# mp3guy/ElasticFusion

Hardware: AMD Instinct MI355X
Metric: frames/s per GPU, 640x480 3-level ICP+fuse (higher is better)
Workload: dtype f32

## Files before the change

### elasticfusion_amd/api.py

```python
from __future__ import annotations

import ctypes as C
import os
import re

import numpy as np

_HERE = os.path.dirname(os.path.abspath(__file__))
LIB_PATH = os.environ.get("EF_HIP_LIB") or os.path.join(_HERE, "libefusion_hip.so")
_lib = None

c_f, c_i, c_u32, P = C.c_float, C.c_int, C.c_uint32, C.c_void_p


class EFError(RuntimeError):
    pass


class ef_config(C.Structure):
    _fields_ = [("width", c_i), ("height", c_i), ("fx", c_f), ("fy", c_f), ("cx", c_f), ("cy", c_f),
                ("time_delta", c_i), ("confidence", c_f), ("depth_cut", c_f), ("icp_weight", c_f),
                ("fast_odom", c_i), ("so3", c_i), ("frame_to_frame_rgb", c_i), ("pyramid", c_i), ("rgb_only", c_i),
                ("close_loops", c_i), ("max_surfels", c_u32), ("device", c_i), ("stream", P)]

# ... 1147 lines not shown

    def _carveArgs(self, depths, poses, params, among, kw):
        T = self.get_T_wc().reshape(1, 16) if poses is None else np.ascontiguousarray(poses, np.float64).reshape(-1, 16)
        if params is None:
            if not isinstance(depths, DevBuf) and "width" not in kw and "height" not in kw:
                kw = dict(kw, width=int(np.shape(depths)[-1]), height=int(np.shape(depths)[-2]))
            params = self.carveParams(**kw)
        else:
            assert not kw, "give params or keywords, not both"
        if isinstance(depths, DevBuf):
            assert len(T) * params.width * params.height * 2 <= depths.nbytes, (len(T), depths.nbytes)
            keep, dp = depths, depths.p
        else:
            keep = np.ascontiguousarray(depths, np.uint16).reshape(-1, params.height, params.width)
            assert len(keep) == len(T), (keep.shape, T.shape)
            dp = _ptr(keep)
        views = ef_carve_views(len(T), _ptr(T), dp)
        if isinstance(among, dict):
            among = self.mapSelection(**among)
        return params, views, (C.byref(among) if among is not None else None), (T, keep, among)

    def carveSelect(self, depths, poses=None, params: ef_carve_params | None = None, among=None, max_rows: int | None = None,
                    count: bool = False, votes: bool = False, **kw):
        params, views, pa, keep = self._carveArgs(depths, poses, params, among, kw)
        n = self.lastCount() if max_rows is None or votes else 0
        cap = n if max_rows is None else int(max_rows)
        rows = np.zeros(max(cap, 1), np.uint32)
        v2 = np.zeros((max(n, 1), 2), np.uint8) if votes else None
        total = c_u32(0)
        _chk(lib().ef_map_carve_select(self.h, C.byref(params), C.byref(views), pa, _ptr(rows) if cap else None, cap, C.byref(total),
                                       _ptr(v2) if votes else None), self.h)
        out = (rows[:min(cap, total.value)].copy(),) + ((total.value,) if count else ()) + ((v2[:n],) if votes else ())
        return out if len(out) > 1 else out[0]

    def carveSelectDevice(self, depths_dev, poses, params: ef_carve_params, among, rows_dev, max_rows: int, count_dev, votes_dev=None):
        T = np.ascontiguousarray(poses, np.float64).reshape(-1, 16)
        if isinstance(among, dict):
            among = self.mapSelection(**among)
        views = ef_carve_views(len(T), _ptr(T), _dev(depths_dev))
        _chk(lib().ef_map_carve_select_dev(self.h, C.byref(params), C.byref(views), C.byref(among) if among is not None else None,
                                           _dev(rows_dev), int(max_rows), _dev(count_dev), _dev(votes_dev)), self.h)

    def carveSurfels(self, depths, poses=None, params: ef_carve_params | None = None, among=None, **kw) -> dict:
        params, views, pa, keep = self._carveArgs(depths, poses, params, among, kw)
        res = ef_carve_result()
        fn = lib().ef_map_carve_dev if isinstance(depths, DevBuf) else lib().ef_map_carve
        _chk(fn(self.h, C.byref(params), C.byref(views), pa, C.byref(res)), self.h)
        return {k: int(getattr(res, k)) for k, _ in ef_carve_result._fields_}

    def setReferenceDownload(self, on=True):
        _chk(lib().ef_set_reference_download(self.h, int(on)), self.h)

    def uploadMap(self, surfels: np.ndarray):
        s = np.ascontiguousarray(surfels, np.float32).reshape(-1, 12)
        _chk(lib().ef_map_upload(self.h, _ptr(s), len(s)), self.h)

    def getPoseQT(self) -> np.ndarray:
        qt = np.zeros(7, np.float64)
        _chk(lib().ef_get_pose_qt(self.h, _ptr(qt)), self.h)
        return qt

    def checkpoint(self, last_rgb, last_depth) -> dict:
        return dict(map=self.downloadMap(), tick=self.getTick(), qt=self.getPoseQT(), rgb=np.ascontiguousarray(last_rgb, np.uint8).copy(),
                    depth=np.ascontiguousarray(last_depth, np.uint16).copy())

    def restore(self, ck: dict):
        self.uploadMap(ck["map"])
        qt = np.ascontiguousarray(ck["qt"], np.float64).reshape(7)
        _chk(lib().ef_restore_state(self.h, int(ck["tick"]), _ptr(qt), _ptr(ck["rgb"]), _ptr(ck["depth"])), self.h)

    def savePly(self, path: str):
        _chk(lib().ef_save_ply(self.h, path.encode()), self.h)

    def saveFreiburg(self, path: str):
        _chk(lib().ef_save_freiburg(self.h, path.encode()), self.h)

    def setRgbOnly(self, v): _chk(lib().ef_set_rgb_only(self.h, int(v)), self.h)
    def setIcpWeight(self, v): _chk(lib().ef_set_icp_weight(self.h, v), self.h)
    def setPyramid(self, v): _chk(lib().ef_set_pyramid(self.h, int(v)), self.h)
    def setFastOdom(self, v): _chk(lib().ef_set_fast_odom(self.h, int(v)), self.h)
    def setSo3(self, v): _chk(lib().ef_set_so3(self.h, int(v)), self.h)
    def setFrameToFrameRGB(self, v): _chk(lib().ef_set_frame_to_frame_rgb(self.h, int(v)), self.h)
    def setConfidenceThreshold(self, v): _chk(lib().ef_set_confidence_threshold(self.h, v), self.h)
    def setDepthCutoff(self, v): _chk(lib().ef_set_depth_cutoff(self.h, v), self.h)
    def setInputOverlap(self, on): _chk(lib().ef_set_input_overlap(self.h, int(on)), self.h)
    def setInputCuMask(self, one_in_n): _chk(lib().ef_set_input_cu_mask(self.h, int(one_in_n)), self.h)
    def setDeformation(self, graph, isFern=False):
        g = np.ascontiguousarray(graph, np.float32).reshape(-1, 16)
        _chk(lib().ef_set_deformation(self.h, _ptr(g), len(g), int(isFern)), self.h)

    def setGraphReplay(self, on): _chk(lib().ef_set_graph_replay(self.h, int(on)), self.h)

    def image(self, name: str) -> np.ndarray:
        which, dt, ch = self.IMAGES[name]
        W, H = self.cfg.width, self.cfg.height
        out = np.zeros((H, W, ch) if ch > 1 else (H, W), dt)
        _chk(lib().ef_get_image(self.h, which, _ptr(out), out.nbytes), self.h)
        return out

    def trackerBuffer(self, name: str, level: int = 0, tracker: int = 0) -> np.ndarray:
        which, dt, planes = self.TRACKER[name]
        w, h = self.cfg.width >> level, self.cfg.height >> level
        out = np.zeros((h * planes, w), dt)
        _chk(lib().ef_get_tracker_buffer_of(self.h, tracker, which, level, _ptr(out), out.nbytes), self.h)
        return out

    def enableTiming(self, on=True):
        _chk(lib().ef_enable_timing(self.h, int(on)), self.h)

    def timings(self) -> dict:
        arr = (ef_timing * 32)()
        n = c_i(0)
        _chk(lib().ef_get_timings(self.h, arr, 32, C.byref(n)), self.h)
        return {arr[i].name.decode(): arr[i].ms for i in range(n.value)}


class ops:
    @staticmethod
    def _f32(a):
        return np.ascontiguousarray(a, np.float32)

    @staticmethod
    def _image_op(name, src, dtype, scale, *scalars):
        h, w = src.shape[:2]
        shape = (h // scale, w // scale)
        s, d = DevBuf.from_array(src), DevBuf(shape[0] * shape[1] * np.dtype(dtype).itemsize)
        _chk(getattr(lib(), "ef_op_" + name)(s.p, w, h, *scalars, d.p, None))
        return d.to_array(dtype, shape)

    @staticmethod
    def pyr_down(src):
        return ops._image_op("pyr_down", src, np.uint16, 2)

    @staticmethod
    def create_vmap(depth, fx, fy, cx, cy, cutoff, init=None):
        h, w = depth.shape
        d = DevBuf.from_array(depth)
        v = DevBuf.from_array(np.zeros((3 * h, w), np.float32) if init is None else init)
        k = ef_intr(fx, fy, cx, cy)
        _chk(lib().ef_op_create_vmap(C.byref(k), d.p, w, h, cutoff, v.p, None))
        return v.to_array(np.float32, (3 * h, w))

    @staticmethod
    def create_nmap(vmap, init=None):
        h3, w = vmap.shape
        v = DevBuf.from_array(vmap)
        n = DevBuf.from_array(np.zeros((h3, w), np.float32) if init is None else init)
        _chk(lib().ef_op_create_nmap(v.p, w, h3 // 3, n.p, None))
        return n.to_array(np.float32, (h3, w))

    @staticmethod
    def transform_maps(vmap, nmap, R, t):
        h3, w = vmap.shape
        v, n = DevBuf.from_array(vmap), DevBuf.from_array(nmap)
        R9, t3 = ops._f32(R).reshape(9), ops._f32(t).reshape(3)
        _chk(lib().ef_op_transform_maps(v.p, n.p, w, h3 // 3, _ptr(R9), _ptr(t3), v.p, n.p, None))
        return v.to_array(np.float32, (h3, w)), n.to_array(np.float32, (h3, w))

    @staticmethod
    def copy_maps(vtex, ntex):
        h, w, _ = vtex.shape
        v4, n4 = DevBuf.from_array(ops._f32(vtex)), DevBuf.from_array(ops._f32(ntex))
        tmp, vm, nm = DevBuf(h * w * 16), DevBuf(h * w * 12), DevBuf(h * w * 12)
        _chk(lib().ef_op_copy_maps(v4.p, n4.p, w, h, tmp.p, vm.p, nm.p, None))
        return tmp.to_array(np.float32, (h, w, 4)), vm.to_array(np.float32, (3 * h, w)), nm.to_array(np.float32, (3 * h, w))

    @staticmethod
    def resize_map(src, normalize, init=None):
        h3, w = src.shape
        s = DevBuf.from_array(src)
        o = DevBuf.from_array(np.zeros((h3 // 2, w // 2), np.float32) if init is None else init)
        fn = lib().ef_op_resize_nmap if normalize else lib().ef_op_resize_vmap
        _chk(fn(s.p, w, h3 // 3, o.p, None))
        return o.to_array(np.float32, (h3 // 2, w // 2))

    @staticmethod
    def pyr_down_gauss_f(src):
        return ops._image_op("pyr_down_gauss_f", src, np.float32, 2)

    @staticmethod
    def pyr_down_uchar_gauss(src):
        return ops._image_op("pyr_down_uchar_gauss", src, np.uint8, 2)

    @staticmethod
    def vertices_to_depth(vmaps_tmp, cutoff):
        return ops._image_op("vertices_to_depth", ops._f32(vmaps_tmp), np.float32, 1, cutoff)

    @staticmethod
    def bgr_to_intensity(rgba):
        return ops._image_op("image_bgr_to_intensity", rgba, np.uint8, 1)

    @staticmethod
    def derivative_images(img):
        h, w = img.shape
        s, dx, dy = DevBuf.from_array(img), DevBuf(h * w * 2), DevBuf(h * w * 2)
        _chk(lib().ef_op_compute_derivative_images(s.p, w, h, dx.p, dy.p, None))
        return dx.to_array(np.int16, (h, w)), dy.to_array(np.int16, (h, w))

    @staticmethod
    def project_to_point_cloud(depth, fx, fy, cx, cy, level=0):
        h, w = depth.shape
        s, d = DevBuf.from_array(depth), DevBuf(h * w * 12)
        k = ef_intr(fx, fy, cx, cy)
        _chk(lib().ef_op_project_to_point_cloud(s.p, w, h, C.byref(k), level, d.p, None))
        return d.to_array(np.float32, (h, w, 3))

    @staticmethod
    def icp_step(Rcurr, tcurr, vmap_curr, nmap_curr, Rprev_inv, tprev, intr, vmap_g_prev, nmap_g_prev, distThres, angleThres):
        h3, w = vmap_curr.shape
        bufs = [DevBuf.from_array(a) for a in (vmap_curr, nmap_curr, vmap_g_prev, nmap_g_prev)]
        A, b, res = np.zeros((6, 6), np.float32), np.zeros(6, np.float32), np.zeros(2, np.float32)
        k = ef_intr(*intr)
        _chk(lib().ef_op_icp_step(_ptr(ops._f32(Rcurr).reshape(9)), _ptr(ops._f32(tcurr)), bufs[0].p, bufs[1].p,
                                  _ptr(ops._f32(Rprev_inv).reshape(9)), _ptr(ops._f32(tprev)), C.byref(k), bufs[2].p, bufs[3].p,
                                  distThres, angleThres, w, h3 // 3, _ptr(A), _ptr(b), _ptr(res), None))
        return A, b, res

    @staticmethod
    def rgb_residual(minScale, dIdx, dIdy, lastDepth, nextDepth, lastImage, nextImage, maxDepthDelta, kt, krkinv):
        h, w = nextImage.shape
        bufs = [DevBuf.from_array(a) for a in (dIdx, dIdy, lastDepth, nextDepth, lastImage, nextImage)]
        corres = DevBuf(h * w * 16)
        sigma, count = c_i(0), c_i(0)
        _chk(lib().ef_op_compute_rgb_residual(minScale, bufs[0].p, bufs[1].p, bufs[2].p, bufs[3].p, bufs[4].p, bufs[5].p, corres.p,
                                              maxDepthDelta, _ptr(ops._f32(kt)), _ptr(ops._f32(krkinv).reshape(9)), w, h,
                                              C.byref(sigma), C.byref(count), None))
        return corres.to_array(DATATERM, (h, w)), sigma.value, count.value

    @staticmethod
    def rgb_step(corres, sigma, cloud, fx, fy, dIdx, dIdy, sobelScale):
        h, w = corres.shape
        bufs = [DevBuf.from_array(a) for a in (corres, ops._f32(cloud), dIdx, dIdy)]
        A, b = np.zeros((6, 6), np.float32), np.zeros(6, np.float32)
        _chk(lib().ef_op_rgb_step(bufs[0].p, sigma, bufs[1].p, fx, fy, bufs[2].p, bufs[3].p, sobelScale, w, h,
                                  _ptr(A), _ptr(b), None))
        return A, b

    @staticmethod
    def so3_step(lastImage, nextImage, imageBasis, kinv, krlr):
        h, w = nextImage.shape
        li, ni = DevBuf.from_array(lastImage), DevBuf.from_array(nextImage)
        A, b, res = np.zeros((3, 3), np.float32), np.zeros(3, np.float32), np.zeros(2, np.float32)
        _chk(lib().ef_op_so3_step(li.p, ni.p, _ptr(ops._f32(imageBasis).reshape(9)), _ptr(ops._f32(kinv).reshape(9)),
                                  _ptr(ops._f32(krlr).reshape(9)), w, h, _ptr(A), _ptr(b), _ptr(res), None))
        return A, b, res

    @staticmethod
    def model_maps(pred_vertex, pred_normal, fill_vertex, fill_normal, R, t, maxDepthRGB=6.0, pred_image=None, fill_image=None, camera_frame=False,
                   force_fill_image=False, tally=False, dense_count=0, dense_samples=1, joint=False, raw=None, rgb=None, depth_cut=3.0, init=None):
        h, w, _ = pred_vertex.shape
        init = init or {}
        keep = [DevBuf.from_array(ops._f32(a)) for a in (pred_vertex, pred_normal, fill_vertex, fill_normal)]
        a = ef_model_maps_op()
        a.cols, a.rows = w, h
        a.pred_vertex, a.pred_normal, a.fill_vertex, a.fill_normal = (b.p for b in keep)
        if pred_image is not None:
            imgs = [DevBuf.from_array(np.ascontiguousarray(i, np.uint8)) for i in (pred_image, fill_image)]
            keep += imgs
            a.pred_image, a.fill_image = imgs[0].p, imgs[1].p
        a.R[:] = [float(v) for v in ops._f32(R).reshape(9)]
        a.t[:] = [float(v) for v in ops._f32(t).reshape(3)]
        a.max_depth_rgb = float(maxDepthRGB)
        a.camera_frame, a.force_fill_image, a.tally = int(camera_frame), int(force_fill_image), int(tally)
        a.dense_count, a.dense_samples = int(dense_count), int(dense_samples)
        spec = {}
        for l in range(3):
            spec[f"vmap{l}"] = spec[f"nmap{l}"] = (np.float32, (3 * (h >> l), w >> l))
        spec["depth0"], spec["last0"] = (np.float32, (h, w)), (np.uint8, (h, w))
        if joint:
            spec.update(filtered=(np.uint16, (h, w)), metric=(np.float32, (h, w)), metric_filtered=(np.float32, (h, w)), next0=(np.uint8, (h, w)))
        out = {}
        for name, (dt, shp) in spec.items():
            start = np.zeros(shp, dt) if name not in init else np.ascontiguousarray(init[name], dt)
            assert start.shape == shp, (name, start.shape, shp)
            out[name] = DevBuf.from_array(start)
        for l in range(3):
            a.vmap[l], a.nmap[l] = out[f"vmap{l}"].p, out[f"nmap{l}"].p
        a.depth0, a.last0 = out["depth0"].p, out["last0"].p
        if joint:
            fr = [DevBuf.from_array(np.ascontiguousarray(raw, np.uint16)), DevBuf.from_array(np.ascontiguousarray(rgb, np.uint8))]
            assert raw.shape == (h, w) and rgb.shape == (h, w, 3)
            keep += fr
            a.joint, a.raw, a.rgb3, a.depth_cut = 1, fr[0].p, fr[1].p, float(depth_cut)
            a.filtered, a.metric, a.metric_filtered, a.next0 = (out[n].p for n in ("filtered", "metric", "metric_filtered", "next0"))
        left = C.c_uint(0)
        _chk(lib().ef_op_model_maps(C.byref(a), C.byref(left), None))
        res = {name: out[name].to_array(*spec[name]) for name in spec}
        res["dense_count"] = int(left.value)
        return res

    @staticmethod
    def sobel_mask(nextImage, nextDepth):
        h, w = nextImage[0].shape
        img = [DevBuf.from_array(np.ascontiguousarray(a, np.uint8)) for a in nextImage]
        dep = [DevBuf.from_array(ops._f32(a)) for a in nextDepth]
        for l in range(3):
            assert nextImage[l].shape == nextDepth[l].shape == (h >> l, w >> l), (l, nextImage[l].shape, nextDepth[l].shape)
        outs = [[DevBuf((h >> l) * (w >> l) * sz, fill=0xA5) for l in range(3)] for sz in (2, 2, 1, 4)]
        arr = lambda bufs: (P * 3)(*[b.p for b in bufs])
        _chk(lib().ef_op_sobel_mask(arr(img), arr(dep), w, h, arr(outs[0]), arr(outs[1]), arr(outs[2]), arr(outs[3]), None))
        return tuple([b.to_array(dt, (h >> l, w >> l)) for l, b in enumerate(bufs)] for bufs, dt in zip(outs, (np.int16, np.int16, np.uint8, np.uint32)))

    @staticmethod
    def clean_deform(cam, T_wc, time, idx, vc, ct, nr, confThreshold, timeDelta, maxDepth, surfels, newUnstable, graph, depth, isFern=0):
        s = ops._f32(surfels).reshape(-1, 12)
        nu = ops._f32(newUnstable).reshape(-1, 12)
        g = ops._f32(graph).reshape(-1, 16)
        bufs = [DevBuf.from_array(a) for a in (idx, ops._f32(vc), ops._f32(ct), ops._f32(nr), g, ops._f32(depth))]
        sb, nb = DevBuf.from_array(s), DevBuf.from_array(nu if len(nu) else np.zeros((1, 12), np.float32))
        out = DevBuf((len(s) + len(nu) + 1) * 48)
        n = c_u32(0)
        _chk(lib().ef_op_clean_deform(C.byref(cam), _ptr(ops._T(T_wc)), time, bufs[0].p, bufs[1].p, bufs[2].p, bufs[3].p,
                                      confThreshold, timeDelta, maxDepth, sb.p, len(s), nb.p, len(nu),
                                      bufs[4].p, len(g), bufs[5].p, int(isFern), out.p, C.byref(n), None))
        return out.to_array(np.float32, (n.value, 12))

    LINALG = dict(ldlt6=0, ldlt3f=1, polar3=2, rodrigues=3, se3_inverse=4, se3_log_norm=5, scalar=6, ldlt6_wave=7, ldlt6_every_lane=8,
                  mat_to_quat=9, se3_mul=10, se3_castf=11, se3_inverse_f=12, m4_affine_inverse=13, ldlt_pivots=14, lu_inverse6=15)

    @staticmethod
    def linalg(which, vec, n_out):
        v = np.ascontiguousarray(np.asarray(vec, np.float64).reshape(-1))
        out = np.zeros(n_out, np.float64)
        _chk(lib().ef_op_linalg(ops.LINALG[which], _ptr(v), v.size, _ptr(out), n_out))
        return out

    GN_STATE = ("Rcurr", "tcurr", "resultRt", "krkinv", "kt", "lastRGBErrorLevel", "rgb_broken")

    @staticmethod
    def gn_update(sums, prev, Rprev, tprev, count, sigma, icp, rgb, rgbOnly, icpWeight, knext, level_changes, split_tail, lastA, lastb, stats):
        a = ef_gn_update_args()
        a.sums[:] = [float(v) for v in ops._f32(sums).reshape(58)]
        for name in ("Rcurr", "tcurr", "krkinv", "kt"):
            getattr(a.prev, name)[:] = [float(v) for v in ops._f32(prev[name]).reshape(-1)]
        a.prev.resultRt[:] = [float(v) for v in np.asarray(prev["resultRt"], np.float64).reshape(16)]
        a.prev.lastRGBErrorLevel, a.prev.rgb_broken = float(np.float32(prev["lastRGBErrorLevel"])), int(prev["rgb_broken"])
        a.Rprev[:] = [float(v) for v in ops._f32(Rprev).reshape(9)]
        a.tprev[:] = [float(v) for v in ops._f32(tprev).reshape(3)]
        a.count, a.sigma, a.icp, a.rgb, a.rgb_only = int(count), int(sigma), int(icp), int(rgb), int(rgbOnly)
        a.icp_weight, a.knext, a.level_changes, a.split_tail = float(icpWeight), ef_intr(*[float(v) for v in knext]), int(level_changes), int(split_tail)
        nxt = ef_gn_state()
        A = np.ascontiguousarray(np.asarray(lastA, np.float64).reshape(36)).copy()
        b = np.ascontiguousarray(np.asarray(lastb, np.float64).reshape(6)).copy()
        st = ops._f32(stats).reshape(4).copy()
        _chk(lib().ef_op_gn_update(C.byref(a), C.byref(nxt), _ptr(A), _ptr(b), _ptr(st)))
        out = {n: np.array(getattr(nxt, n)) for n in ("Rcurr", "tcurr", "resultRt", "krkinv", "kt")}
        out["lastRGBErrorLevel"], out["rgb_broken"] = np.float32(nxt.lastRGBErrorLevel), int(nxt.rgb_broken)
        return out, A, b, st

    @staticmethod
    def track_end_tail(Rcurr, tcurr, Rprev, tprev, q_prev, t_prev, rgb, weightMultiplier):
        o = ef_track_end_out()
        qp = np.ascontiguousarray(np.asarray(q_prev, np.float64).reshape(4))
        tp = np.ascontiguousarray(np.asarray(t_prev, np.float64).reshape(3))
        _chk(lib().ef_op_track_end_tail(_ptr(ops._f32(Rcurr).reshape(9)), _ptr(ops._f32(tcurr).reshape(3)), _ptr(ops._f32(Rprev).reshape(9)),
                                        _ptr(ops._f32(tprev).reshape(3)), _ptr(qp), _ptr(tp), int(rgb), weightMultiplier, C.byref(o)))
        out = {n: np.array(getattr(o, n)) for n in ("q", "t", "logged", "T_cw", "pose_f", "R_wc_f", "t_wc_f")}
        out["weighting"] = np.float32(o.weighting)
        return out

    @staticmethod
    def filter_depth(raw, maxD):
        return ops._image_op("filter_depth", raw, np.uint16, 1, maxD)

    @staticmethod
    def metricise_depth(d_in, maxD):
        return ops._image_op("metricise_depth", d_in, np.float32, 1, maxD)

    @staticmethod
    def seed_map(cam, rgb, dm, dmf, time, maxDepth):
        Pn = cam.cols * cam.rows
        bufs = [DevBuf.from_array(a) for a in (rgb, dm, dmf)]
        out = DevBuf(Pn * 48)
        n = c_u32(0)
        _chk(lib().ef_op_seed_map(C.byref(cam), bufs[0].p, bufs[1].p, bufs[2].p, time, maxDepth, out.p, C.byref(n), None))
        return out.to_array(np.float32, (n.value, 12))

    @staticmethod
    def _T(T):
        return np.ascontiguousarray(T, np.float64).reshape(16)

    @staticmethod
    def predict_indices(cam, T_wc, time, surfels, maxDepth, timeDelta):
        s = ops._f32(surfels).reshape(-1, 12)
        Pn = cam.cols * cam.rows
        sb = DevBuf.from_array(s)
        idx, vc, ct, nr = DevBuf(Pn * 4), DevBuf(Pn * 16), DevBuf(Pn * 16), DevBuf(Pn * 16)
        _chk(lib().ef_op_predict_indices(C.byref(cam), _ptr(ops._T(T_wc)), time, sb.p, len(s), maxDepth, timeDelta,
                                         idx.p, vc.p, ct.p, nr.p, None))
        shp = (cam.rows, cam.cols)
        return (idx.to_array(np.uint32, shp), vc.to_array(np.float32, shp + (4,)), ct.to_array(np.float32, shp + (4,)),
                nr.to_array(np.float32, shp + (4,)))

    @staticmethod
    def combined_predict(cam, T_wc, surfels, maxDepth, confThreshold, time, maxTime, timeDelta):
        s = ops._f32(surfels).reshape(-1, 12)
        Pn = cam.cols * cam.rows
        sb = DevBuf.from_array(s)
        img, vt, nm, tm = DevBuf(Pn * 4), DevBuf(Pn * 16), DevBuf(Pn * 16), DevBuf(Pn * 2)
        _chk(lib().ef_op_combined_predict(C.byref(cam), _ptr(ops._T(T_wc)), sb.p, len(s), maxDepth, confThreshold,
                                          time, maxTime, timeDelta, img.p, vt.p, nm.p, tm.p, None))
        shp = (cam.rows, cam.cols)
        return (img.to_array(np.uint8, shp + (4,)), vt.to_array(np.float32, shp + (4,)), nm.to_array(np.float32, shp + (4,)),
                tm.to_array(np.uint16, shp))

    @staticmethod
    def synthesize_depth(cam, T_wc, surfels, maxDepth, confThreshold, time, maxTime, timeDelta):
        s = ops._f32(surfels).reshape(-1, 12)
        Pn = cam.cols * cam.rows
        sb, d = DevBuf.from_array(s), DevBuf(Pn * 4)
        _chk(lib().ef_op_synthesize_depth(C.byref(cam), _ptr(ops._T(T_wc)), sb.p, len(s), maxDepth, confThreshold,
                                          time, maxTime, timeDelta, d.p, None))
        return d.to_array(np.float32, (cam.rows, cam.cols))

    @staticmethod
    def fill_in(cam, image, vertex, normal, depthFiltered, rgb, passthrough=0, passthroughImage=0):
        bufs = [DevBuf.from_array(a) for a in (image, ops._f32(vertex), ops._f32(normal), depthFiltered, rgb)]
        Pn = cam.cols * cam.rows
        fi, fv, fn = DevBuf(Pn * 4), DevBuf(Pn * 16), DevBuf(Pn * 16)
        _chk(lib().ef_op_fill_in(C.byref(cam), bufs[0].p, bufs[1].p, bufs[2].p, bufs[3].p, bufs[4].p, passthrough, passthroughImage,
                                 fi.p, fv.p, fn.p, None))
        shp = (cam.rows, cam.cols)
        return fi.to_array(np.uint8, shp + (4,)), fv.to_array(np.float32, shp + (4,)), fn.to_array(np.float32, shp + (4,))

    @staticmethod
    def dense_enough(cam, image):
        b = DevBuf.from_array(image)
        d = c_i(0)
        _chk(lib().ef_op_dense_enough(C.byref(cam), b.p, C.byref(d), None))
        return bool(d.value)

    @staticmethod
    def fuse(cam, T_wc, time, rgb, dm, dmf, idx, vc, ct, nr, maxDepth, weighting, surfels):
        s = ops._f32(surfels).reshape(-1, 12)
        bufs = [DevBuf.from_array(a) for a in (rgb, dm, dmf, idx, ops._f32(vc), ops._f32(ct), ops._f32(nr))]
        sb = DevBuf.from_array(s)
        nu = DevBuf((cam.cols // 2) * (cam.rows // 2) * 48)
        n = c_u32(0)
        _chk(lib().ef_op_fuse(C.byref(cam), _ptr(ops._T(T_wc)), time, bufs[0].p, bufs[1].p, bufs[2].p, bufs[3].p, bufs[4].p, bufs[5].p,
                              bufs[6].p, maxDepth, weighting, sb.p, len(s), nu.p, C.byref(n), None))
        return sb.to_array(np.float32, (len(s), 12)), nu.to_array(np.float32, (n.value, 12))

    @staticmethod
    def clean(cam, T_wc, time, idx, vc, ct, nr, confThreshold, timeDelta, maxDepth, surfels, newUnstable):
        s = ops._f32(surfels).reshape(-1, 12)
        nu = ops._f32(newUnstable).reshape(-1, 12)
        bufs = [DevBuf.from_array(a) for a in (idx, ops._f32(vc), ops._f32(ct), ops._f32(nr))]
        sb, nb = DevBuf.from_array(s), DevBuf.from_array(nu if len(nu) else np.zeros((1, 12), np.float32))
        out = DevBuf((len(s) + len(nu) + 1) * 48)
        n = c_u32(0)
        _chk(lib().ef_op_clean(C.byref(cam), _ptr(ops._T(T_wc)), time, bufs[0].p, bufs[1].p, bufs[2].p, bufs[3].p, confThreshold,
                               timeDelta, maxDepth, sb.p, len(s), nb.p, len(nu), out.p, C.byref(n), None))
        return out.to_array(np.float32, (n.value, 12))
```

### elasticfusion_amd/csrc/ef_host_ops.inc

```
extern "C" {

__global__ void k_calib_empty() {}
__global__ void __launch_bounds__(256) k_calib_stream(const float4* __restrict__ src, float4* __restrict__ dst, int n) {
  for (int i = blockIdx.x * blockDim.x + threadIdx.x; i < n; i += gridDim.x * blockDim.x) dst[i] = src[i];
}
int ef_dev_calibrate(void* stream, float* empty_us, float* stream16mb_us) {
  if (!empty_us || !stream16mb_us) return EF_EINVAL;
  hipStream_t s = (hipStream_t)stream;
  const int n = 1 << 20, reps = 200;
  float4 *a = nullptr, *b = nullptr;
  hipEvent_t e0 = nullptr, e1 = nullptr;
  int rc = EF_EHIP;
  float ms = 0;
  if (hipMalloc((void**)&a, (size_t)n * sizeof(float4)) != hipSuccess || hipMalloc((void**)&b, (size_t)n * sizeof(float4)) != hipSuccess) { rc = EF_ENOMEM; goto done; }
  if (hipMemsetAsync(a, 0, (size_t)n * sizeof(float4), s) != hipSuccess) goto done;
  if (hipEventCreate(&e0) != hipSuccess || hipEventCreate(&e1) != hipSuccess) goto done;
  for (int pass = 0; pass < 2; ++pass) {
    if (hipEventRecord(e0, s) != hipSuccess) goto done;
    for (int i = 0; i < reps; ++i) hipLaunchKernelGGL(k_calib_empty, dim3(256), dim3(256), 0, s);
    if (hipEventRecord(e1, s) != hipSuccess || hipEventSynchronize(e1) != hipSuccess || hipEventElapsedTime(&ms, e0, e1) != hipSuccess) goto done;
    *empty_us = 1e3f * ms / reps;
    if (hipEventRecord(e0, s) != hipSuccess) goto done;
    for (int i = 0; i < reps; ++i) hipLaunchKernelGGL(k_calib_stream, dim3(2048), dim3(256), 0, s, (const float4*)a, b, n);
    if (hipEventRecord(e1, s) != hipSuccess || hipEventSynchronize(e1) != hipSuccess || hipEventElapsedTime(&ms, e0, e1) != hipSuccess) goto done;
    *stream16mb_us = 1e3f * ms / reps;
  }
  rc = EF_OK;
done:
  if (e0) (void)hipEventDestroy(e0);
  if (e1) (void)hipEventDestroy(e1);
  if (a) (void)hipFree(a);
  if (b) (void)hipFree(b);
  return rc;
}

int ef_dev_alloc(void** dev, size_t bytes) { return hipMalloc(dev, bytes ? bytes : 1) == hipSuccess ? EF_OK : EF_ENOMEM; }
int ef_dev_free(void* dev) { return hipFree(dev) == hipSuccess ? EF_OK : EF_EHIP; }
int ef_dev_upload(void* dev, const void* host, size_t bytes) { return hipMemcpy(dev, host, bytes, hipMemcpyHostToDevice) == hipSuccess ? EF_OK : EF_EHIP; }
int ef_dev_download(void* host, const void* dev, size_t bytes) { return hipMemcpy(host, dev, bytes, hipMemcpyDeviceToHost) == hipSuccess ? EF_OK : EF_EHIP; }
int ef_dev_memset(void* dev, int value, size_t bytes) { return hipMemset(dev, value, bytes) == hipSuccess ? EF_OK : EF_EHIP; }
int ef_dev_sync(void) { return hipDeviceSynchronize() == hipSuccess ? EF_OK : EF_EHIP; }
int ef_device_count(int* n) { return hipGetDeviceCount(n) == hipSuccess ? EF_OK : EF_EHIP; }
int ef_set_device(int d) { return hipSetDevice(d) == hipSuccess ? EF_OK : EF_EHIP; }

#define OP_TAIL(s)                                                         \
  do {                                                                     \
    hipError_t _e = hipGetLastError();                                     \
    if (_e != hipSuccess) { g_create_error = hipGetErrorString(_e); return EF_EHIP; } \
    return EF_OK;                                                          \
  } while (0)
#define OP_SYNC(s)                                                         \
  do {                                                                     \
    hipError_t _e = hipStreamSynchronize((hipStream_t)(s));                \
    if (_e == hipSuccess) _e = hipGetLastError();                          \
    if (_e != hipSuccess) { g_create_error = hipGetErrorString(_e); return EF_EHIP; } \
  } while (0)

int ef_op_pyr_down(const uint16_t* src, int sc, int sr, uint16_t* dst, void* s) { eft::pyr_down_u16(src, sc, sr, dst, (hipStream_t)s); OP_TAIL(s); }
int ef_op_create_vmap(const ef_intr* k, const uint16_t* depth, int cols, int rows, float cutoff, float* vmap, void* s) {
  eft::create_vmap(depth, cols, rows, eft::Intr{k->fx, k->fy, k->cx, k->cy}, cutoff, vmap, (hipStream_t)s);
  OP_TAIL(s);
}
int ef_op_create_nmap(const float* vmap, int cols, int rows, float* nmap, void* s) { eft::create_nmap(vmap, cols, rows, nmap, (hipStream_t)s); OP_TAIL(s); }
int ef_op_transform_maps(const float* vs, const float* ns, int cols, int rows, const float* R9, const float* t3, float* vd, float* nd, void* s) {
  float* rt = nullptr;
  if (hipMalloc((void**)&rt, 12 * sizeof(float)) != hipSuccess) return EF_ENOMEM;
  float h[12];
  memcpy(h, R9, 36);
  memcpy(h + 9, t3, 12);
  (void)hipMemcpyAsync(rt, h, sizeof(h), hipMemcpyHostToDevice, (hipStream_t)s);
  eft::transform_maps(vs, ns, cols, rows, rt, rt + 9, vd, nd, (hipStream_t)s);
  (void)hipStreamSynchronize((hipStream_t)s);
  (void)hipFree(rt);
  OP_TAIL(s);
}
int ef_op_copy_maps(const float* v4, const float* n4, int cols, int rows, float* tmp, float* vd, float* nd, void* s) {
  eft::copy_maps(v4, n4, cols, rows, tmp, vd, nd, (hipStream_t)s);
  OP_TAIL(s);
}
int ef_op_resize_vmap(const float* in, int sc, int sr, float* out, void* s) { eft::resize_map(in, sc, sr, out, false, (hipStream_t)s); OP_TAIL(s); }
int ef_op_resize_nmap(const float* in, int sc, int sr, float* out, void* s) { eft::resize_map(in, sc, sr, out, true, (hipStream_t)s); OP_TAIL(s); }
int ef_op_pyr_down_gauss_f(const float* src, int sc, int sr, float* dst, void* s) { eft::pyr_down_gauss_f(src, sc, sr, dst, (hipStream_t)s); OP_TAIL(s); }
int ef_op_pyr_down_uchar_gauss(const uint8_t* src, int sc, int sr, uint8_t* dst, void* s) { eft::pyr_down_uchar_gauss(src, sc, sr, dst, (hipStream_t)s); OP_TAIL(s); }
int ef_op_vertices_to_depth(const float* tmp, int cols, int rows, float cutoff, float* dst, void* s) { eft::vertices_to_depth(tmp, cols, rows, cutoff, dst, (hipStream_t)s); OP_TAIL(s); }
int ef_op_image_bgr_to_intensity(const uint8_t* rgba, int cols, int rows, uint8_t* dst, void* s) { eft::bgr_to_intensity(rgba, 4, cols, rows, dst, (hipStream_t)s); OP_TAIL(s); }
int ef_op_compute_derivative_images(const uint8_t* src, int cols, int rows, int16_t* dx, int16_t* dy, void* s) {
  eft::derivative_images(src, cols, rows, dx, dy, (hipStream_t)s);
  OP_TAIL(s);
}
int ef_op_project_to_point_cloud(const float* depth, int cols, int rows, const ef_intr* k0, int level, float* cloud, void* s) {
  eft::project_to_point_cloud(depth, cols, rows, eft::intr_level(eft::Intr{k0->fx, k0->fy, k0->cx, k0->cy}, level), cloud, (hipStream_t)s);
  OP_TAIL(s);
}

static int op_scratch(float** partials, float** out, int nfloats_out) {
  if (hipMalloc((void**)partials, (size_t)eft::OP_SCRATCH_FLOATS * sizeof(float)) != hipSuccess) return EF_ENOMEM;
  if (hipMalloc((void**)out, nfloats_out * sizeof(float)) != hipSuccess) { (void)hipFree(*partials); return EF_ENOMEM; }
  return EF_OK;
}
static void unpack29_host(const float* h, float* A, float* b) {
  int shift = 0;
  for (int i = 0; i < 6; ++i)
    for (int j = i; j < 7; ++j) {
      const float v = h[shift++];
      if (j == 6) b[i] = v;
      else A[j * 6 + i] = A[i * 6 + j] = v;
    }
}
int ef_op_icp_step(const float* Rc, const float* tc, const float* vc, const float* nc, const float* Rpi, const float* tp, const ef_intr* k,
                   const float* vg, const float* ng, float dist, float ang, int cols, int rows, float* A, float* b, float* res, void* s) {
  if (cols <= 0 || rows <= 0 || cols > 2048 || rows > 2048) return EF_EINVAL;
  eft::IcpArgs a;
  memcpy(a.Rcurr, Rc, 36); memcpy(a.tcurr, tc, 12); memcpy(a.Rprev_inv, Rpi, 36); memcpy(a.tprev, tp, 12);
  a.k = eft::Intr{k->fx, k->fy, k->cx, k->cy};
  a.distThres = dist; a.angleThres = ang;
  float *partials, *out;
  int r = op_scratch(&partials, &out, 32);
  if (r != EF_OK) return r;
  eft::icp_step_op(a, vc, nc, vg, ng, cols, rows, partials, out, (hipStream_t)s);
  float h[32];
  (void)hipMemcpyAsync(h, out, 29 * sizeof(float), hipMemcpyDeviceToHost, (hipStream_t)s);
  hipError_t e = hipStreamSynchronize((hipStream_t)s);
  (void)hipFree(partials); (void)hipFree(out);
  if (e != hipSuccess) { g_create_error = hipGetErrorString(e); return EF_EHIP; }
  unpack29_host(h, A, b);
  res[0] = h[27]; res[1] = h[28];
  return EF_OK;
}
int ef_op_compute_rgb_residual(float minScale, const int16_t* dIdx, const int16_t* dIdy, const float* lastDepth, const float* nextDepth,
                               const uint8_t* lastImage, const uint8_t* nextImage, void* corres, float maxDepthDelta, const float* kt,
                               const float* krkinv, int cols, int rows, int* sigma, int* count, void* s) {
  eft::RgbResidualArgs a;
  a.minScale = minScale; a.maxDepthDelta = maxDepthDelta;
  memcpy(a.kt, kt, 12); memcpy(a.krkinv, krkinv, 36);
  int* out;
  if (hipMalloc((void**)&out, 2 * sizeof(int)) != hipSuccess) return EF_ENOMEM;
  eft::rgb_residual_op(a, dIdx, dIdy, lastDepth, nextDepth, lastImage, nextImage, corres, cols, rows, out, (hipStream_t)s);
  int h[2] = {0, 0};
  hipError_t e = hipMemcpy(h, out, sizeof(h), hipMemcpyDeviceToHost);
  (void)hipFree(out);
  if (e != hipSuccess) { g_create_error = hipGetErrorString(e); return EF_EHIP; }
  *count = h[0];
  *sigma = h[1];
  return EF_OK;
}
int ef_op_rgb_step(const void* corres, float sigma, const float* cloud, float fx, float fy, const int16_t* dIdx, const int16_t* dIdy,
                   float sobelScale, int cols, int rows, float* A, float* b, void* s) {
  float *partials, *out;
  int r = op_scratch(&partials, &out, 32);
  if (r != EF_OK) return r;
  eft::rgb_step_op(corres, sigma, cloud, fx, fy, dIdx, dIdy, sobelScale, cols, rows, partials, out, (hipStream_t)s);
  float h[32];
  (void)hipMemcpyAsync(h, out, 29 * sizeof(float), hipMemcpyDeviceToHost, (hipStream_t)s);
  hipError_t e = hipStreamSynchronize((hipStream_t)s);
  (void)hipFree(partials); (void)hipFree(out);
  if (e != hipSuccess) { g_create_error = hipGetErrorString(e); return EF_EHIP; }
  unpack29_host(h, A, b);
  return EF_OK;
}
int ef_op_so3_step(const uint8_t* lastImage, const uint8_t* nextImage, const float* ib, const float* kinv, const float* krlr, int cols,
                   int rows, float* A, float* b, float* res, void* s) {
  eft::So3Args a;
  memcpy(a.imageBasis, ib, 36); memcpy(a.kinv, kinv, 36); memcpy(a.krlr, krlr, 36);
  float *partials, *out;
  int r = op_scratch(&partials, &out, 16);
  if (r != EF_OK) return r;
  eft::so3_step_op(a, lastImage, nextImage, cols, rows, partials, out, (hipStream_t)s);
  float h[11];
  (void)hipMemcpyAsync(h, out, sizeof(h), hipMemcpyDeviceToHost, (hipStream_t)s);
  hipError_t e = hipStreamSynchronize((hipStream_t)s);
  (void)hipFree(partials); (void)hipFree(out);
  if (e != hipSuccess) { g_create_error = hipGetErrorString(e); return EF_EHIP; }
  int shift = 0;
  for (int i = 0; i < 3; ++i)
    for (int j = i; j < 4; ++j) {
      const float v = h[shift++];
      if (j == 3) b[i] = v;
      else A[j * 3 + i] = A[i * 3 + j] = v;
    }
  res[0] = h[9]; res[1] = h[10];
  return EF_OK;
}

int ef_op_model_maps(const ef_model_maps_op* a, unsigned* dense_count_left, void* s) {
  if (!a || !dense_count_left || a->cols <= 0 || a->rows <= 0 || a->cols > 2048 || a->rows > 2048 || (a->cols & 3) || (a->rows & 3)) return EF_EINVAL;
  if (!a->pred_vertex || !a->pred_normal || !a->fill_vertex || !a->fill_normal || !a->depth0) return EF_EINVAL;
  if ((a->pred_image == nullptr) != (a->fill_image == nullptr) || (a->pred_image && !a->last0)) return EF_EINVAL;
  for (int i = 0; i < eft::NUM_PYRS; ++i)
    if (!a->vmap[i] || !a->nmap[i]) return EF_EINVAL;
  if (a->joint && (!a->raw || !a->rgb3 || !a->filtered || !a->metric || !a->metric_filtered || !a->next0)) return EF_EINVAL;
  eft::ModelMapsOp o{};
  o.cols = a->cols; o.rows = a->rows;
  o.pred_vertex = a->pred_vertex; o.pred_normal = a->pred_normal; o.fill_vertex = a->fill_vertex; o.fill_normal = a->fill_normal;
  o.pred_image = a->pred_image; o.fill_image = a->fill_image;
  memcpy(o.R, a->R, 36); memcpy(o.t, a->t, 12);
  o.maxDepthRGB = a->max_depth_rgb;
  o.camera_frame = a->camera_frame != 0; o.force_fill_image = a->force_fill_image != 0; o.tally = a->tally != 0;
  o.dense_count = a->dense_count; o.dense_samples = a->dense_samples;
  for (int i = 0; i < eft::NUM_PYRS; ++i) { o.vmap[i] = a->vmap[i]; o.nmap[i] = a->nmap[i]; }
  o.depth0 = a->depth0; o.last0 = a->last0;
  eft::FramePreprocess fp{};
  if (a->joint) {
    fp = eft::FramePreprocess{a->raw, a->depth_cut, efm::bilateral_table(), a->filtered, a->metric, a->metric_filtered, a->rgb3, nullptr};
    if (!fp.table) { g_create_error = "bilateral weight table missing on this device"; return EF_EHIP; }
    o.with = &fp; o.next0 = a->next0;
  }
  const hipError_t e = (hipError_t)eft::model_maps_op(o, dense_count_left, (hipStream_t)s);
  if (e != hipSuccess) { g_create_error = hipGetErrorString(e); return e == hipErrorOutOfMemory ? EF_ENOMEM : EF_EHIP; }
  return EF_OK;
}
int ef_op_sobel_mask(const uint8_t* const* nextImage, const float* const* nextDepth, int cols, int rows, int16_t* const* dIdx, int16_t* const* dIdy,
                     uint8_t* const* mask, uint32_t* const* corres, void* s) {
  if (!nextImage || !nextDepth || !dIdx || !dIdy || !mask || !corres || cols <= 0 || rows <= 0 || cols > 2048 || rows > 2048) return EF_EINVAL;
  eft::SobelMaskOp o{};
  o.cols = cols; o.rows = rows;
  for (int i = 0; i < eft::NUM_PYRS; ++i) {
    if (!nextImage[i] || !nextDepth[i] || !dIdx[i] || !dIdy[i] || !mask[i] || !corres[i]) return EF_EINVAL;
    o.nextImage[i] = nextImage[i]; o.nextDepth[i] = nextDepth[i]; o.dIdx[i] = dIdx[i]; o.dIdy[i] = dIdy[i]; o.mask[i] = mask[i]; o.corres[i] = corres[i];
  }
  eft::sobel_mask_op(o, (hipStream_t)s);
  const hipError_t le = hipGetLastError();
  if (le != hipSuccess) { g_create_error = hipGetErrorString(le); return EF_EHIP; }
  OP_SYNC(s);
  return EF_OK;
}

}
namespace {
__global__ void k_linalg_probe(int which, const double* __restrict__ in, double* __restrict__ out) {
  if (which == EF_LINALG_LDLT6_WAVE || which == EF_LINALG_LDLT6_EVERY_LANE) {
    __shared__ efs::SolveScratch S;
    const int lane = threadIdx.x;
    if (lane < 6) S.b[lane] = in[36 + lane];
    efs::wave_sync();
    if (which == EF_LINALG_LDLT6_WAVE) efs::ldlt6_wave(in[lane < 36 ? lane : 0], S);
    else efs::ldlt6_every_lane(in[lane < 36 ? lane : 0], S);
    if (lane < 6) out[lane] = S.x[lane];
    return;
  }
  if (threadIdx.x != 0) return;
  switch (which) {
    case EF_LINALG_LDLT6: efl::ldlt_solve<double, 6>(in, in + 36, out); break;
    case EF_LINALG_LDLT3F: {
      float A[9], b[3], x[3];
      for (int i = 0; i < 9; ++i) A[i] = (float)in[i];
      for (int i = 0; i < 3; ++i) b[i] = (float)in[9 + i];
      efl::ldlt_solve<float, 3>(A, b, x);
      for (int i = 0; i < 3; ++i) out[i] = (double)x[i];
      break;
    }
    case EF_LINALG_POLAR3: efl::polar3(in, out); break;
    case EF_LINALG_RODRIGUES: efl::rodrigues(in, out); break;
    case EF_LINALG_SE3_INVERSE: efl::se3_matrix(efl::se3_inverse(efl::se3_from_matrix(in)), out); break;
    case EF_LINALG_SE3_LOG_NORM: out[0] = efl::se3_log_norm(efl::se3_from_matrix(in)); break;
    case EF_LINALG_SCALAR:
      out[0] = sqrt(in[0]); out[1] = in[0] / in[1]; out[2] = sin(in[0]); out[3] = cos(in[0]); out[4] = atan2(in[0], in[1]);
      break;
    case EF_LINALG_MAT_TO_QUAT: {
      efl::mat_to_quat(in, out);
      efl::SE3 T;
      efl::se3_set_rotation(T, in);
      for (int i = 0; i < 4; ++i) out[4 + i] = T.q[i];
      break;
    }
    case EF_LINALG_SE3_MUL: {
      const efl::SE3 T = efl::se3_mul(efl::se3_from_matrix(in), efl::se3_from_matrix(in + 16));
      for (int i = 0; i < 4; ++i) out[i] = T.q[i];
      for (int i = 0; i < 3; ++i) out[4 + i] = T.t[i];
      break;
    }
    case EF_LINALG_SE3_CASTF:
    case EF_LINALG_SE3_INVERSE_F: {
      float M[16];
      if (which == EF_LINALG_SE3_CASTF) efl::se3_castf_matrix(efl::se3_from_matrix(in), M);
      else efl::se3_inverse_matrix_f(efl::se3_from_matrix(in), M);
      for (int i = 0; i < 16; ++i) out[i] = (double)M[i];
      break;
    }
    case EF_LINALG_M4_AFFINE_INVERSE: efl::m4_affine_inverse(in, out); break;
    case EF_LINALG_LDLT_PIVOTS: efl::ldlt_pivots<double, 6>(in, out); break;
    case EF_LINALG_LU_INVERSE6: efl::lu_inverse<double, 6>(in, out); break;
    default: break;
  }
}
}
extern "C" {
int ef_op_linalg(int which, const double* in, int n_in, double* out, int n_out) {
  if (!in || !out || n_in <= 0 || n_out <= 0 || n_in > 64 || n_out > 64 || which < 0 || which > EF_LINALG_LU_INVERSE6) return EF_EINVAL;
  double* d;
  if (hipMalloc((void**)&d, 128 * sizeof(double)) != hipSuccess) return EF_ENOMEM;
  (void)hipMemset(d, 0, 128 * sizeof(double));
  (void)hipMemcpy(d, in, n_in * sizeof(double), hipMemcpyHostToDevice);
  hipLaunchKernelGGL(k_linalg_probe, dim3(1), dim3(64), 0, 0, which, (const double*)d, d + 64);
  hipError_t e = hipMemcpy(out, d + 64, n_out * sizeof(double), hipMemcpyDeviceToHost);
  (void)hipFree(d);
  if (e != hipSuccess) { g_create_error = hipGetErrorString(e); return EF_EHIP; }
  return EF_OK;
}

static_assert(sizeof(ef_gn_state) == sizeof(eft::GNState), "ef_gn_state is eft::GNState");
int ef_op_gn_update(const ef_gn_update_args* in, ef_gn_state* next, double* lastA36, double* lastb6, float* stats4) {
  if (!in || !next || !lastA36 || !lastb6 || !stats4 || !(in->icp || in->rgb)) return EF_EINVAL;
  eft::GnUpdateProbe p;
  memcpy(p.sums, in->sums, sizeof(p.sums));
  memcpy(&p.prev, &in->prev, sizeof(p.prev));
  memcpy(p.Rprev, in->Rprev, 36); memcpy(p.tprev, in->tprev, 12);
  p.count = in->count; p.sigma = in->sigma;
  p.icp = in->icp != 0; p.rgb = in->rgb != 0; p.rgbOnly = in->rgb_only != 0;
  p.icpWeight = in->icp_weight;
  p.knext = eft::Intr{in->knext.fx, in->knext.fy, in->knext.cx, in->knext.cy};
  p.level_changes = in->level_changes != 0;
  p.split_tail = in->split_tail != 0;
  const hipError_t e = (hipError_t)eft::gn_update_op(p, (eft::GNState*)next, lastA36, lastb6, stats4);
  if (e != hipSuccess) { g_create_error = hipGetErrorString(e); return e == hipErrorOutOfMemory ? EF_ENOMEM : EF_EHIP; }
  return EF_OK;
}
int ef_op_track_end_tail(const float* Rcurr9, const float* tcurr3, const float* Rprev9, const float* tprev3, const double* q_prev4,
                         const double* t_prev3, int rgb, float weight_multiplier, ef_track_end_out* out) {
  if (!Rcurr9 || !tcurr3 || !Rprev9 || !tprev3 || !q_prev4 || !t_prev3 || !out) return EF_EINVAL;
  eft::TrackState* st = new eft::TrackState();
  memcpy(st->Rprev, Rprev9, 36); memcpy(st->tprev, tprev3, 12);
  memcpy(st->q_prev, q_prev4, 32); memcpy(st->t_prev, t_prev3, 24);
  float pose[12];
  memcpy(pose, Rcurr9, 36); memcpy(pose + 9, tcurr3, 12);
  const hipError_t e = (hipError_t)eft::track_end_tail_op(st, pose, rgb != 0, weight_multiplier, out->logged);
  if (e == hipSuccess) {
    memcpy(out->q, st->q, 32); memcpy(out->t, st->t, 24);
    memcpy(out->T_cw, st->T_cw, 64); memcpy(out->pose_f, st->pose_f, 64);
    memcpy(out->R_wc_f, st->R_wc_f, 36); memcpy(out->t_wc_f, st->t_wc_f, 12);
    out->weighting = st->weighting;
  }
  delete st;
  if (e != hipSuccess) { g_create_error = hipGetErrorString(e); return e == hipErrorOutOfMemory ? EF_ENOMEM : EF_EHIP; }
  return EF_OK;
}

int ef_op_filter_depth(const uint16_t* raw, int cols, int rows, float maxD, uint16_t* filtered, void* s) {
  if (!efm::filter_depth(raw, cols, rows, maxD, filtered, (hipStream_t)s)) return EF_EHIP;
  OP_TAIL(s);
}
int ef_op_metricise_depth(const uint16_t* in, int cols, int rows, float maxD, float* out, void* s) {
  efm::metricise_depth(in, cols, rows, maxD, out, (hipStream_t)s);
  OP_TAIL(s);
}

}
namespace {
struct OpMap {
  std::vector<void*> allocs;
  template <typename T>
  T* alloc(size_t n, int fill = 0) {
    void* p = nullptr;
    if (hipMalloc(&p, (n ? n : 1) * sizeof(T)) != hipSuccess) return nullptr;
    (void)hipMemset(p, fill, (n ? n : 1) * sizeof(T));
    allocs.push_back(p);
    return (T*)p;
  }
  efm::SurfelSoA soa(size_t n) { return efm::SurfelSoA{alloc<float4>(n), alloc<float4>(n), alloc<float4>(n)}; }
  ~OpMap() { for (void* p : allocs) (void)hipFree(p); }
};
efm::Cam to_cam(const ef_cam* c) { return efm::Cam{c->cols, c->rows, c->fx, c->fy, c->cx, c->cy}; }
}
extern "C" {

int ef_op_seed_map(const ef_cam* cam, const uint8_t* rgb, const float* dm, const float* dmf, int time, float maxDepth, float* surfels,
                   uint32_t* count_host, void* s_) {
  hipStream_t s = (hipStream_t)s_;
  OpMap m;
  const size_t P = (size_t)cam->cols * cam->rows;
  efm::SurfelSoA soa = m.soa(P);
  efm::CompactScratch cs;
  cs.max_chunks = (int)(2 * P / efm::CHUNK + 8);
  cs.flags = m.alloc<uint8_t>(2 * P);
  cs.chunk_count = m.alloc<uint32_t>(cs.max_chunks);
  cs.chunk_offset = m.alloc<uint32_t>(cs.max_chunks);
  cs.totals = m.alloc<uint32_t>(8);
  unsigned* cnt = m.alloc<unsigned>(1);
  efm::seed_map(to_cam(cam), rgb, dm, dmf, time, maxDepth, soa, cnt, cs, s);
  unsigned h = 0;
  (void)hipMemcpyAsync(&h, cnt, sizeof(h), hipMemcpyDeviceToHost, s);
  OP_SYNC(s);
  efm::soa_to_aos(soa, h, surfels, s);
  OP_SYNC(s);
  *count_host = h;
  return EF_OK;
}

int ef_op_predict_indices(const ef_cam* cam, const double* T16, int time, const float* surfels, uint32_t count, float maxDepth, int timeDelta,
                          uint32_t* index, float* vc, float* ct, float* nr, void* s_) {
  hipStream_t s = (hipStream_t)s_;
  OpMap m;
  const size_t P = (size_t)cam->cols * cam->rows;
  efm::SurfelSoA soa = m.soa(count);
  efm::aos_to_soa(surfels, count, soa, s);
  float h[32];
  pose_mats(T16, h, h + 16);
  float* mats = m.alloc<float>(32);
  (void)hipMemcpyAsync(mats, h, sizeof(h), hipMemcpyHostToDevice, s);
  unsigned* cnt = m.alloc<unsigned>(1);
  (void)hipMemcpyAsync(cnt, &count, sizeof(unsigned), hipMemcpyHostToDevice, s);
  unsigned long long* zbuf = m.alloc<unsigned long long>(P, 0xFF);
  efm::IndexMaps im{index, (float4*)vc, (float4*)ct, (float4*)nr};
  efm::predict_indices(to_cam(cam), mats, time, soa, cnt, maxDepth, timeDelta, zbuf, im, s);
  OP_SYNC(s);
  return EF_OK;
}

int ef_op_combined_predict(const ef_cam* cam, const double* T16, const float* surfels, uint32_t count, float maxDepth, float confThreshold,
                           int time, int maxTime, int timeDelta, uint8_t* image, float* vertex, float* normal, uint16_t* timeMap, void* s_) {
  hipStream_t s = (hipStream_t)s_;
  OpMap m;
  const size_t P = (size_t)cam->cols * cam->rows;
  efm::SurfelSoA soa = m.soa(count);
  efm::aos_to_soa(surfels, count, soa, s);
  float h[32];
  pose_mats(T16, h, h + 16);
  float* mats = m.alloc<float>(32);
  (void)hipMemcpyAsync(mats, h, sizeof(h), hipMemcpyHostToDevice, s);
  unsigned* cnt = m.alloc<unsigned>(1);
  (void)hipMemcpyAsync(cnt, &count, sizeof(unsigned), hipMemcpyHostToDevice, s);
  unsigned long long* zbuf = m.alloc<unsigned long long>(P, 0xFF);
  efm::PredictMaps pm{(uchar4*)image, (float4*)vertex, (float4*)normal, timeMap};
  efm::FillMaps none{nullptr, nullptr, nullptr};
  efm::combined_predict(to_cam(cam), mats, soa, cnt, maxDepth, confThreshold, time, maxTime, timeDelta, zbuf, pm, none, nullptr, nullptr, false,
                        nullptr, s);
  OP_SYNC(s);
  return EF_OK;
}

int ef_op_synthesize_depth(const ef_cam* cam, const double* T16, const float* surfels, uint32_t count, float maxDepth, float confThreshold,
                           int time, int maxTime, int timeDelta, float* depth, void* s_) {
  hipStream_t s = (hipStream_t)s_;
  OpMap m;
  const size_t P = (size_t)cam->cols * cam->rows;
  efm::SurfelSoA soa = m.soa(count);
  efm::aos_to_soa(surfels, count, soa, s);
  float h[32];
  pose_mats(T16, h, h + 16);
  float* mats = m.alloc<float>(32);
  (void)hipMemcpyAsync(mats, h, sizeof(h), hipMemcpyHostToDevice, s);
  unsigned* cnt = m.alloc<unsigned>(1);
  (void)hipMemcpyAsync(cnt, &count, sizeof(unsigned), hipMemcpyHostToDevice, s);
  unsigned long long* zbuf = m.alloc<unsigned long long>(P, 0xFF);
  efm::synthesize_depth(to_cam(cam), mats, soa, cnt, maxDepth, confThreshold, time, maxTime, timeDelta, zbuf, depth, s);
  OP_SYNC(s);
  return EF_OK;
}

int ef_op_fill_in(const ef_cam* cam, const uint8_t* image, const float* vertex, const float* normal, const uint16_t* depthFiltered,
                  const uint8_t* rgb, int passthrough, int passthroughImage, uint8_t* fimage, float* fvertex, float* fnormal, void* s_) {
  efm::PredictMaps pm{(uchar4*)image, (float4*)vertex, (float4*)normal, nullptr};
  efm::FillMaps fm{(uchar4*)fimage, (float4*)fvertex, (float4*)fnormal};
  efm::fill_in(to_cam(cam), pm, depthFiltered, rgb, passthrough != 0, passthroughImage != 0, fm, (hipStream_t)s_);
  OP_TAIL(s_);
}

int ef_op_dense_enough(const ef_cam* cam, const uint8_t* image, int* dense_host, void* s_) {
  hipStream_t s = (hipStream_t)s_;
  OpMap m;
  unsigned* cnt = m.alloc<unsigned>(1);
  efm::dense_count(to_cam(cam), (const uchar4*)image, cnt, s);
  unsigned h = 0;
  (void)hipMemcpyAsync(&h, cnt, sizeof(h), hipMemcpyDeviceToHost, s);
  OP_SYNC(s);
  *dense_host = ((float)h / (float)((cam->cols / 20) * (cam->rows / 20)) > 0.75f) ? 1 : 0;
  return EF_OK;
}

int ef_op_fuse(const ef_cam* cam, const double* T16, int time, const uint8_t* rgb, const float* dm, const float* dmf, const uint32_t* index,
               const float* vc, const float* ct, const float* nr, float maxDepth, float weighting, float* surfels, uint32_t count,
               float* newUnstable, uint32_t* newCount, void* s_) {
  hipStream_t s = (hipStream_t)s_;
  OpMap m;
  efm::SurfelSoA soa = m.soa(count);
  efm::aos_to_soa(surfels, count, soa, s);
  float h[33];
  pose_mats(T16, h, h + 16);
  h[32] = weighting;
  float* mats = m.alloc<float>(33);
  (void)hipMemcpyAsync(mats, h, sizeof(h), hipMemcpyHostToDevice, s);
  unsigned* cnt = m.alloc<unsigned>(2);
  (void)hipMemcpyAsync(cnt, &count, sizeof(unsigned), hipMemcpyHostToDevice, s);
  efm::Candidates cand;
  cand.n = (cam->cols / 2) * (cam->rows / 2);
  cand.pos_conf = m.alloc<float4>(cand.n);
  cand.col_time = m.alloc<float4>(cand.n);
  cand.nrm_rad = m.alloc<float4>(cand.n);
  cand.best = m.alloc<uint32_t>(cand.n);
  uint32_t* winner = m.alloc<uint32_t>(count, 0xFF);
  efm::IndexMaps im{(uint32_t*)index, (float4*)vc, (float4*)ct, (float4*)nr};
  efm::fuse(to_cam(cam), mats + 16, time, rgb, dm, dmf, im, maxDepth, mats + 32, soa, cnt, cand, winner, s);
  efm::soa_to_aos(soa, count, surfels, s);
  efm::CompactScratch cs;
  cs.max_chunks = cand.n / efm::CHUNK + 8;
  cs.flags = m.alloc<uint8_t>(cand.n);
  cs.chunk_count = m.alloc<uint32_t>(cs.max_chunks);
  cs.chunk_offset = m.alloc<uint32_t>(cs.max_chunks);
  cs.totals = m.alloc<uint32_t>(8);
  efm::candidates_to_aos(cand, newUnstable, cnt + 1, cs, s);
  unsigned hn = 0;
  (void)hipMemcpyAsync(&hn, cnt + 1, sizeof(hn), hipMemcpyDeviceToHost, s);
  OP_SYNC(s);
  *newCount = hn;
  return EF_OK;
}

}
namespace {
__global__ void k_aos_to_cand(const float4* __restrict__ aos, uint32_t n, efm::Candidates cand) {
  const uint32_t i = blockIdx.x * blockDim.x + threadIdx.x;
  if (i >= (uint32_t)cand.n) return;
  if (i < n) {
    cand.pos_conf[i] = aos[(size_t)i * 3];
    cand.col_time[i] = aos[(size_t)i * 3 + 1];
    cand.nrm_rad[i] = aos[(size_t)i * 3 + 2];
  } else {
    cand.col_time[i] = make_float4(0, 0, 0, 0);
  }
}
}
extern "C" {

int ef_op_clean_deform(const ef_cam* cam, const double* T16, int time, const uint32_t* index, const float* vc, const float* ct, const float* nr,
// ... 50 lines not shown
```

### elasticfusion_amd/csrc/ef_track.hpp

```cpp
#pragma once
#include <hip/hip_runtime.h>
#include <stdint.h>

#include "ef_build.hpp"

namespace eft {

constexpr int NUM_PYRS = 3;
constexpr int REDUCE_BLOCK = 256;
constexpr int VTHREADS = 16384;
constexpr int VWARPS = VTHREADS / 32;
constexpr int RGB_SLOTS = 64;
constexpr int SE3_ACCS = 29;
constexpr int SO3_ACCS = 11;
constexpr int SE3_PAIRS = VWARPS / 2;
constexpr int PARTIAL_FLOATS = 2 * SE3_ACCS * SE3_PAIRS > SO3_ACCS * VWARPS ? 2 * SE3_ACCS * SE3_PAIRS : SO3_ACCS * VWARPS;
constexpr int PT_WGS = 128, PT_BLOCK = 512, PT_MAX_ITER = 16, PT_MAX_PIXELS = 8 * VTHREADS, PT_SYNC_FLOATS = 1024;
constexpr int PARTIAL_ALLOC_FLOATS = (2 * PARTIAL_FLOATS + PT_SYNC_FLOATS) > 196608 ? (2 * PARTIAL_FLOATS + PT_SYNC_FLOATS) : 196608;
constexpr int FT_EPOCHS = 64;

struct Intr { float fx, fy, cx, cy; };
__host__ __device__ inline Intr intr_level(const Intr& k, int level) {
  const int div = 1 << level;
  return Intr{k.fx / div, k.fy / div, k.cx / div, k.cy / div};
}

struct GNState {
  float Rcurr[9], tcurr[3];
  double resultRt[16];
  float krkinv[9], kt[3];
  float lastRGBErrorLevel;
  int rgb_broken;
};

struct TrackState {
  double q[4];
  double t[3];
  double q_prev[4];
  double t_prev[3];
  float Rprev[9], tprev[3], Rprev_inv[9];
  GNState gn[2];
  int rgb_slots[2][RGB_SLOTS][16];
  float lastICPError, lastICPCount, lastRGBError, lastRGBCount, lastSO3Error, lastSO3Count;
  double lastA[36], lastb[6];
  int so3_iterations;
  double so3_resultR[9], so3_lastResultR[9];
  float so3_R_lr[9];
  float so3_mats[27];
  float so3_lastError, so3_lastCount;
  int so3_done;
  unsigned so3_ticket;
  float weighting;
  unsigned dense_count;
  int dense_samples;
  int tick;
  unsigned long long step_rec[16];
  unsigned call_seq;
  unsigned step_timeout;
  unsigned long long dbg_clock[16];
  unsigned map_counts[2];
  unsigned model_view_stamp;
  float T_cw[16];
  float pose_f[16];
  float R_wc_f[9], t_wc_f[3];
};

struct TrackerPlan {
  int script = 0;
  int n_small = 0;
  int n_iter = 0;
  unsigned long long levels = 0;
  unsigned res_bytes = 0;
  unsigned res_budget = 0;
};

struct Pyramid {
  int width, height;
  uint16_t* depth_tmp[NUM_PYRS];
  float* vmap_curr[NUM_PYRS];
  float* nmap_curr[NUM_PYRS];
  float* vmap_g_prev[NUM_PYRS];
  float* nmap_g_prev[NUM_PYRS];
  float* lastDepth[NUM_PYRS];
  float* nextDepth[NUM_PYRS];
  uint8_t* lastImage[NUM_PYRS];
  uint8_t* nextImage[NUM_PYRS];
  uint8_t* lastNextImage[NUM_PYRS];
  int16_t* dIdx[NUM_PYRS];
  int16_t* dIdy[NUM_PYRS];
  uint32_t* corres[NUM_PYRS];
  uint8_t* rgbMask[NUM_PYRS];
  float* partials;
  unsigned epoch = 1;
  int last_mode = 0;
  unsigned sticky_abort = 0, fallbacks_base = 0;
  TrackerPlan plan;
  int W(int l) const { return width >> l; }
  int H(int l) const { return height >> l; }
};

struct KernelProbe {
  hipEvent_t* start;
  hipEvent_t* stop;
  int capacity;
  int used;
};

struct TrackParams {
  bool rgbOnly, pyramid, fastOdom, so3;
  float icpWeight;
  float distThres, angleThres;
  int fused_step = 0;
  int persistent = 1;
  const unsigned* empty_model_flag = nullptr;
  unsigned empty_model_value = 0;
  int no_resident = 0;
};
static_assert(sizeof(TrackParams) == 4 + 4 + 8 + 4 + 4 + 8 + 4 + 4, "TrackParams has no padding bytes (it is compared with memcmp)");

void pyr_down_u16(const uint16_t* src, int scols, int srows, uint16_t* dst, hipStream_t s);
void create_vmap(const uint16_t* depth, int cols, int rows, Intr k, float cutoff, float* vmap, hipStream_t s);
void create_nmap(const float* vmap, int cols, int rows, float* nmap, hipStream_t s);
void transform_maps(const float* vsrc, const float* nsrc, int cols, int rows, const float* R9_dev, const float* t3_dev,
                    float* vdst, float* ndst, hipStream_t s);
void copy_maps(const float* vtex, const float* ntex, int cols, int rows, float* vmaps_tmp, float* vmap, float* nmap, hipStream_t s);
void resize_map(const float* in, int scols, int srows, float* out, bool normalize, hipStream_t s);
void pyr_down_gauss_f(const float* src, int scols, int srows, float* dst, hipStream_t s);
void pyr_down_uchar_gauss(const uint8_t* src, int scols, int srows, uint8_t* dst, hipStream_t s);
void vertices_to_depth(const float* vmaps_tmp, int cols, int rows, float cutoff, float* dst, hipStream_t s);
void bgr_to_intensity(const uint8_t* src, int channels, int cols, int rows, uint8_t* dst, hipStream_t s);
void derivative_images(const uint8_t* src, int cols, int rows, int16_t* dx, int16_t* dy, hipStream_t s);
void project_to_point_cloud(const float* depth, int cols, int rows, Intr k, float* cloud, hipStream_t s);

struct IcpArgs {
  float Rcurr[9], tcurr[3], Rprev_inv[9], tprev[3];
  Intr k;
  float distThres, angleThres;
};
constexpr int OP_SCRATCH_FLOATS = SE3_ACCS * VWARPS + 64;
void icp_step_op(const IcpArgs& a, const float* vmap_curr, const float* nmap_curr, const float* vmap_g_prev,
                 const float* nmap_g_prev, int cols, int rows, float* scratch, float* out29_dev, hipStream_t s);
struct RgbResidualArgs {
  float minScale, maxDepthDelta;
  float kt[3], krkinv[9];
};
void rgb_residual_op(const RgbResidualArgs& a, const int16_t* dIdx, const int16_t* dIdy, const float* lastDepth,
                     const float* nextDepth, const uint8_t* lastImage, const uint8_t* nextImage, void* corres, int cols,
                     int rows, int* out2_dev, hipStream_t s);
void rgb_step_op(const void* corres, float sigma, const float* cloud, float fx, float fy, const int16_t* dIdx,
                 const int16_t* dIdy, float sobelScale, int cols, int rows, float* scratch, float* out29_dev, hipStream_t s);
struct So3Args { float imageBasis[9], kinv[9], krlr[9]; };
void so3_step_op(const So3Args& a, const uint8_t* lastImage, const uint8_t* nextImage, int cols, int rows, float* scratch,
                 float* out11_dev, hipStream_t s);

struct GnUpdateProbe {
  float sums[2 * SE3_ACCS];
  GNState prev;
  float Rprev[9], tprev[3];
  int count, sigma;
  bool icp, rgb, rgbOnly;
  float icpWeight;
  Intr knext;
  bool level_changes;
  bool split_tail;
};
int gn_update_op(const GnUpdateProbe& p, GNState* next_host, double* lastA36, double* lastb6, float* stats4);
int track_end_tail_op(TrackState* st_host, const float* pose12, bool rgb, float weightMultiplier, double* logged16);

struct FramePreprocess {
  const uint16_t* raw;
  float maxD;
  const float* table;
  uint16_t* filtered;
  float* metric;
  float* metric_filtered;
  const uint8_t* rgb3;
  uint8_t* rgb_keep;
};
void init_icp_model(const Pyramid& p, const float* pred_vertex, const float* pred_normal, const float* fill_vertex,
                    const float* fill_normal, const TrackState* st, float maxDepthRGB, hipStream_t s, const uint8_t* pred_image_rgba = nullptr,
                    const uint8_t* fill_image_rgba = nullptr, bool frameToFrameRGB = false, const FramePreprocess* with = nullptr,
                    bool tally = false );
void init_icp_maps(const Pyramid& p, const float* vertex4, const float* normal4, const uint8_t* image_rgba, const TrackState* st,
                   float maxDepthRGB, hipStream_t s);
void build_pyramids(const Pyramid& p, const uint16_t* depth_filtered, Intr k, float cutoff, hipStream_t s, bool with_sobel);
void build_pyramids_frame_side(const Pyramid& p, const uint16_t* depth_filtered, Intr k, float cutoff, hipStream_t s);
void build_pyramids_model_side(const Pyramid& p, hipStream_t s);
void init_rgb_sobel(const Pyramid& p, hipStream_t s);
void init_model_pair(const Pyramid& p, const float* model_vertex4, const float* model_normal4, const uint8_t* model_image_rgba,
                     const float* cur_vertex4, const float* cur_normal4, const uint8_t* cur_image_rgba, const TrackState* st, float maxDepthRGB,
                     hipStream_t s);
struct ModelMapsOp {
  int cols, rows;
  const float *pred_vertex, *pred_normal, *fill_vertex, *fill_normal;
  const uint8_t *pred_image, *fill_image;
  float R[9], t[3], maxDepthRGB;
  bool camera_frame, force_fill_image, tally;
  unsigned dense_count;
  int dense_samples;
  float* vmap[NUM_PYRS];
  float* nmap[NUM_PYRS];
  float* depth0;
  uint8_t* last0;
  const FramePreprocess* with;
  uint8_t* next0;
};
int model_maps_op(const ModelMapsOp& o, unsigned* dense_count_left, hipStream_t s);
struct SobelMaskOp {
  int cols, rows;
  const uint8_t* nextImage[NUM_PYRS];
  const float* nextDepth[NUM_PYRS];
  int16_t* dIdx[NUM_PYRS];
  int16_t* dIdy[NUM_PYRS];
  uint8_t* mask[NUM_PYRS];
  uint32_t* corres[NUM_PYRS];
};
void sobel_mask_op(const SobelMaskOp& o, hipStream_t s);
void init_first_rgb(const Pyramid& p, const uint8_t* rgb3, hipStream_t s);
struct TrackTail {
  int cur, slots;
  bool has_head, icp, rgb, rgbOnly;
  float icpWeight;
  Intr k0;
  const float* pairs;
  int ng = 0;
  bool merged_end = false;
  unsigned epoch = 0;
  float* partials = nullptr;
};
TrackTail track(Pyramid& p, TrackState* st, Intr k, const TrackParams& tp, hipStream_t s, KernelProbe* probe = nullptr,
                KernelProbe* probe_all = nullptr);
int tracker_aborted(const Pyramid& p, hipStream_t s);
void track_prepare(Pyramid& p, const TrackParams& tp, hipStream_t s);
int tracker_fallbacks(const Pyramid& p, hipStream_t s);
void persistent_chain_forget(hipStream_t s);
int tracker_small_clocks(const Pyramid& p, unsigned long long* out32, hipStream_t s);
void track_swap(Pyramid& p, const TrackParams& tp);
void track_end(TrackState* st, const TrackTail& tail, bool rgb, float weightMultiplier, double* traj, int slot, hipStream_t s,
               const unsigned* abort_word = nullptr, unsigned* abort_report = nullptr);
unsigned* tracker_abort_word(const Pyramid& p);
void pose_injected(TrackState* st, const double* T_wc16, bool save_prev, float weightMultiplier, bool with_weighting, double* traj,
                   int slot, hipStream_t s);
void log_pose(const TrackState* st, double* traj, int slot, hipStream_t s);
void pose_restored(TrackState* st, const double* q4, const double* t3, hipStream_t s);
void copy_pose(TrackState* dst, const TrackState* src, hipStream_t s);
void adopt_pose(TrackState* st, const TrackState* est, double* traj, int slot, hipStream_t s);
void sample_constraints(const float* vertex4, const uint16_t* old_time, int cols, int rows, int step, float* out4, hipStream_t s);

}
```

### elasticfusion_amd/csrc/ef_track_host_inputs.inc

```
namespace {
inline dim3 model_maps_grid(const Pyramid& p) {
  return dim3(ceil_div(p.W(0), 64), ceil_div(p.H(0) / 4, 4));
}
ModelMapsArgs model_maps_args(const Pyramid& p, bool model_side, const float* vertex, const float* normal, float maxDepthRGB) {
  ModelMapsArgs A{};
  A.pred_vertex = A.fill_vertex = (const float4*)vertex;
  A.pred_normal = A.fill_normal = (const float4*)normal;
  for (int i = 0; i < NUM_PYRS; ++i) {
    A.vmap[i] = model_side ? p.vmap_g_prev[i] : p.vmap_curr[i];
    A.nmap[i] = model_side ? p.nmap_g_prev[i] : p.nmap_curr[i];
  }
  A.depth0 = model_side ? p.lastDepth[0] : p.nextDepth[0];
  A.cols = p.W(0); A.rows = p.H(0);
  A.maxDepthRGB = maxDepthRGB;
  A.camera_frame = !model_side;
  return A;
}
struct PyrJob { const void* src; void* dst; int type; };
enum { PYR_U16 = 0, PYR_F32 = 1, PYR_U8 = 2 };
void launch_pyr_step(const Pyramid& p, int i, std::initializer_list<PyrJob> jobs, hipStream_t s) {
  PyrJobs J{};
  int n = 0;
  for (const PyrJob& j : jobs) { J.src[n] = j.src; J.dst[n] = j.dst; J.type[n] = j.type; ++n; }
  J.scols = p.W(i); J.srows = p.H(i);
  dim3 g = tile_grid(p.W(i + 1), p.H(i + 1));
  g.z = n;
  hipLaunchKernelGGL(k_pyr_down_multi, g, tile_block(), 0, s, J);
}
inline const uint16_t* frame_depth(const Pyramid& p, const uint16_t* depth_filtered, int i) { return i == 0 ? depth_filtered : p.depth_tmp[i]; }

SobelLevels sobel_levels_of(const Pyramid& p) {
  SobelLevels L;
  const float minGrad[NUM_PYRS] = {5, 3, 1};
  const float sobelScale = 1.0f / 8.0f;
  for (int i = 0; i < NUM_PYRS; ++i) {
    L.src[i] = p.nextImage[i]; L.dx[i] = p.dIdx[i]; L.dy[i] = p.dIdy[i];
    L.nextDepth[i] = p.nextDepth[i]; L.mask[i] = p.rgbMask[i]; L.corres[i] = p.corres[i];
    L.minScale[i] = (float)(pow((double)minGrad[i], 2.0) / pow((double)sobelScale, 2.0));
    L.cols[i] = p.W(i); L.rows[i] = p.H(i);
  }
  return L;
}
void build_vn_levels(const Pyramid& p, const uint16_t* depth_filtered, Intr k, float cutoff, bool with_sobel, hipStream_t s) {
  VNLevels L;
  for (int i = 0; i < NUM_PYRS; ++i) {
    L.depth[i] = frame_depth(p, depth_filtered, i);
    L.vmap[i] = p.vmap_curr[i];
    L.nmap[i] = p.nmap_curr[i];
    L.cols[i] = p.W(i);
    L.rows[i] = p.H(i);
    L.k[i] = intr_level(k, i);
  }
  L.cutoff = cutoff;
  dim3 g = tile_grid(p.W(0), p.H(0));
  if (with_sobel) {
    g.z = 2 * NUM_PYRS;
    hipLaunchKernelGGL(k_vn_sobel_levels, g, tile_block(), 0, s, L, sobel_levels_of(p));
    return;
  }
  g.z = NUM_PYRS;
  hipLaunchKernelGGL(k_vmap_nmap_levels, g, tile_block(), 0, s, L);
}
ModelMapsArgs model_maps_choice_args(const Pyramid& p, bool model_side, const float* pred_vertex, const float* pred_normal, const float* fill_vertex,
                                     const float* fill_normal, const TrackState* st, float maxDepthRGB, const uint8_t* pred_image_rgba,
                                     const uint8_t* fill_image_rgba, bool frameToFrameRGB, bool tally) {
  ModelMapsArgs A = model_maps_args(p, model_side, pred_vertex, pred_normal, maxDepthRGB);
  A.fill_vertex = (const float4*)fill_vertex; A.fill_normal = (const float4*)fill_normal;
  A.pred_image = pred_image_rgba; A.fill_image = fill_image_rgba; A.force_fill_image = frameToFrameRGB;
  A.tally_image = (tally && pred_image_rgba) ? pred_image_rgba : nullptr;
  A.tally_out = const_cast<unsigned*>(&st->dense_count);
  A.last0 = pred_image_rgba ? p.lastImage[0] : nullptr;
  return A;
}
void launch_model_maps(const Pyramid& p, const ModelMapsArgs& A, const TrackState* st, const FramePreprocess* with, hipStream_t s) {
  const dim3 mg = model_maps_grid(p);
  if (with) {
    PreArgs P{};
    P.raw = with->raw; P.cols = p.W(0); P.rows = p.H(0); P.maxv = (unsigned)(with->maxD * 1000.0f); P.table = with->table;
    P.filtered = with->filtered; P.metric = with->metric; P.metric_filtered = with->metric_filtered;
    P.rgb3 = with->rgb3; P.next0 = p.nextImage[0]; P.rgb_keep = with->rgb_keep;
    P.tiles_x = (P.cols + pre::PRE_TW - 1) / pre::PRE_TW;
    P.tiles = P.tiles_x * ((P.rows + pre::PRE_TH - 1) / pre::PRE_TH);
    P.mm_x = (int)mg.x;
    hipLaunchKernelGGL(k_frame_inputs, dim3(P.tiles + (int)(mg.x * mg.y)), dim3(64, 4), 0, s, P, A, st);
    return;
  }
  hipLaunchKernelGGL(k_model_maps, mg, dim3(64, 4), 0, s, A, st);
}
}

void init_icp_model(const Pyramid& p, const float* pred_vertex, const float* pred_normal, const float* fill_vertex,
                    const float* fill_normal, const TrackState* st, float maxDepthRGB, hipStream_t s, const uint8_t* pred_image_rgba,
                    const uint8_t* fill_image_rgba, bool frameToFrameRGB, const FramePreprocess* with, bool tally) {
  launch_model_maps(p, model_maps_choice_args(p, true, pred_vertex, pred_normal, fill_vertex, fill_normal, st, maxDepthRGB, pred_image_rgba,
                                               fill_image_rgba, frameToFrameRGB, tally), st, with, s);
}
int model_maps_op(const ModelMapsOp& o, unsigned* dense_count_left, hipStream_t s) {
  Pyramid p{};
  p.width = o.cols; p.height = o.rows;
  for (int i = 0; i < NUM_PYRS; ++i) {
    p.vmap_g_prev[i] = p.vmap_curr[i] = o.vmap[i];
    p.nmap_g_prev[i] = p.nmap_curr[i] = o.nmap[i];
  }
  p.lastDepth[0] = p.nextDepth[0] = o.depth0;
  p.lastImage[0] = o.last0;
  p.nextImage[0] = o.next0;
  TrackState* h = new TrackState();
  for (int i = 0; i < 9; ++i) h->R_wc_f[i] = o.R[i];
  for (int i = 0; i < 3; ++i) h->t_wc_f[i] = o.t[i];
  h->dense_count = o.dense_count;
  h->dense_samples = o.dense_samples;
  TrackState* st = nullptr;
  hipError_t e = hipMalloc((void**)&st, sizeof(TrackState));
  if (e == hipSuccess) e = hipMemcpy(st, h, sizeof(TrackState), hipMemcpyHostToDevice);
  if (e == hipSuccess) {
    launch_model_maps(p, model_maps_choice_args(p, !o.camera_frame, o.pred_vertex, o.pred_normal, o.fill_vertex, o.fill_normal, st, o.maxDepthRGB,
                                                 o.pred_image, o.fill_image, o.force_fill_image, o.tally), st, o.with, s);
    e = hipGetLastError();
  }
  if (e == hipSuccess) e = hipStreamSynchronize(s);
  if (e == hipSuccess) e = hipMemcpy(dense_count_left, &st->dense_count, sizeof(unsigned), hipMemcpyDeviceToHost);
  if (st) (void)hipFree(st);
  delete h;
  return (int)e;
}
void init_icp_maps(const Pyramid& p, const float* vertex, const float* normal, const uint8_t* image_rgba, const TrackState* st,
                   float maxDepthRGB, hipStream_t s) {
  hipLaunchKernelGGL(k_model_maps, model_maps_grid(p), dim3(64, 4), 0, s, model_maps_args(p, false, vertex, normal, maxDepthRGB), st);
  const int n = p.W(0) * p.H(0);
  for (int i = 0; i + 1 < NUM_PYRS; ++i) pyr_down_gauss_f(p.nextDepth[i], p.W(i), p.H(i), p.nextDepth[i + 1], s);
  hipLaunchKernelGGL(k_model_intensity, dim3(ceil_div(n, 256)), dim3(256), 0, s, image_rgba, image_rgba, true, st, n, p.nextImage[0]);
  for (int i = 0; i + 1 < NUM_PYRS; ++i) pyr_down_uchar_gauss(p.nextImage[i], p.W(i), p.H(i), p.nextImage[i + 1], s);
}
void init_model_pair(const Pyramid& p, const float* model_vertex, const float* model_normal, const uint8_t* model_image_rgba, const float* cur_vertex,
                     const float* cur_normal, const uint8_t* cur_image_rgba, const TrackState* st, float maxDepthRGB, hipStream_t s) {
  hipLaunchKernelGGL(k_model_maps, model_maps_grid(p), dim3(64, 4), 0, s, model_maps_args(p, true, model_vertex, model_normal, maxDepthRGB), st);
  hipLaunchKernelGGL(k_model_maps, model_maps_grid(p), dim3(64, 4), 0, s, model_maps_args(p, false, cur_vertex, cur_normal, maxDepthRGB), st);
  const int n = p.W(0) * p.H(0);
  hipLaunchKernelGGL(k_rgba_intensity_pair, dim3(ceil_div(n, 256), 2), dim3(256), 0, s, model_image_rgba, cur_image_rgba, n, p.lastImage[0], p.nextImage[0]);
  for (int i = 0; i + 1 < NUM_PYRS; ++i)
    launch_pyr_step(p, i, {{p.lastDepth[i], p.lastDepth[i + 1], PYR_F32}, {p.nextDepth[i], p.nextDepth[i + 1], PYR_F32},
                           {p.lastImage[i], p.lastImage[i + 1], PYR_U8}, {p.nextImage[i], p.nextImage[i + 1], PYR_U8}}, s);
}
void build_pyramids(const Pyramid& p, const uint16_t* depth_filtered, Intr k, float cutoff, hipStream_t s, bool with_sobel) {
  for (int i = 0; i + 1 < NUM_PYRS; ++i)
    launch_pyr_step(p, i, {{frame_depth(p, depth_filtered, i), p.depth_tmp[i + 1], PYR_U16}, {p.lastDepth[i], p.lastDepth[i + 1], PYR_F32},
                           {p.lastImage[i], p.lastImage[i + 1], PYR_U8}, {p.nextImage[i], p.nextImage[i + 1], PYR_U8}}, s);
  build_vn_levels(p, depth_filtered, k, cutoff, with_sobel, s);
}
void build_pyramids_frame_side(const Pyramid& p, const uint16_t* depth_filtered, Intr k, float cutoff, hipStream_t s) {
  for (int i = 0; i + 1 < NUM_PYRS; ++i)
    launch_pyr_step(p, i, {{frame_depth(p, depth_filtered, i), p.depth_tmp[i + 1], PYR_U16}, {p.nextImage[i], p.nextImage[i + 1], PYR_U8}}, s);
  build_vn_levels(p, depth_filtered, k, cutoff, false, s);
}
void build_pyramids_model_side(const Pyramid& p, hipStream_t s) {
  for (int i = 0; i + 1 < NUM_PYRS; ++i)
    launch_pyr_step(p, i, {{p.lastDepth[i], p.lastDepth[i + 1], PYR_F32}, {p.lastImage[i], p.lastImage[i + 1], PYR_U8}}, s);
}
void init_rgb_sobel(const Pyramid& p, hipStream_t s) {
  dim3 g = tile_grid(p.W(0), p.H(0));
  g.z = NUM_PYRS;
  hipLaunchKernelGGL(k_sobel_levels, g, tile_block(), 0, s, sobel_levels_of(p));
}
void sobel_mask_op(const SobelMaskOp& o, hipStream_t s) {
  Pyramid p{};
  p.width = o.cols; p.height = o.rows;
  for (int i = 0; i < NUM_PYRS; ++i) {
    p.nextImage[i] = const_cast<uint8_t*>(o.nextImage[i]); p.nextDepth[i] = const_cast<float*>(o.nextDepth[i]);
    p.dIdx[i] = o.dIdx[i]; p.dIdy[i] = o.dIdy[i]; p.rgbMask[i] = o.mask[i]; p.corres[i] = o.corres[i];
  }
  init_rgb_sobel(p, s);
}

void init_first_rgb(const Pyramid& p, const uint8_t* rgb3, hipStream_t s) {
  bgr_to_intensity(rgb3, 3, p.W(0), p.H(0), p.lastNextImage[0], s);
  for (int i = 0; i + 1 < NUM_PYRS; ++i) pyr_down_uchar_gauss(p.lastNextImage[i], p.W(i), p.H(i), p.lastNextImage[i + 1], s);
}
```

### elasticfusion_amd/csrc/ef_track_kernels.hip

```cpp
#include "ef_device.hpp"
#include "ef_linalg_dev.hpp"
#include "ef_solve_dev.hpp"
#include <stddef.h>
#include <initializer_list>
#include <mutex>
#include <type_traits>
#include <hip/hip_ext.h>
#include "ef_track.hpp"

using namespace ef;

namespace eft {

namespace {

constexpr int TILE_X = 64, TILE_Y = 4;

inline dim3 tile_grid(int cols, int rows) { return dim3((cols + TILE_X - 1) / TILE_X, (rows + TILE_Y - 1) / TILE_Y); }
inline dim3 tile_block() { return dim3(TILE_X, TILE_Y); }


__device__ __forceinline__ void pyr_down_u16_px(const uint16_t* __restrict__ src, int scols, int srows, uint16_t* __restrict__ dst, int x, int y) {
  const int dcols = scols / 2;
  const int D = 5;
  const float sigma_color = 30.f;
  int vals[D * D];
#pragma unroll
  for (int yi = -D / 2; yi <= D / 2; ++yi)
#pragma unroll
    for (int xi = -D / 2; xi <= D / 2; ++xi)
      vals[(yi + D / 2) * D + xi + D / 2] = src[min(max(2 * y + yi, 0), srows - 1) * scols + min(max(2 * x + xi, 0), scols - 1)];
  const int center = vals[(D / 2) * D + D / 2];
  float sum = 0, wall = 0;
#pragma unroll
  for (int yi = -D / 2; yi <= D / 2; ++yi)
#pragma unroll
    for (int xi = -D / 2; xi <= D / 2; ++xi) {
      const bool in = 2 * x + xi >= 0 && 2 * x + xi < scols && 2 * y + yi >= 0 && 2 * y + yi < srows;
      const int val = vals[(yi + D / 2) * D + xi + D / 2];
      if (in && abs(val - center) < 3 * sigma_color) {
        const int ax = abs(xi), ay = abs(yi);
        const float wx = ax == 0 ? 0.375f : (ax == 1 ? 0.25f : 0.0625f);
        const float wy = ay == 0 ? 0.375f : (ay == 1 ? 0.25f : 0.0625f);
        sum += (float)val * wx * wy;
        wall += wx * wy;
      }
    }
  dst[y * dcols + x] = (uint16_t) static_cast<int>(sum / wall);
}
__global__ void k_pyr_down_u16(const uint16_t* __restrict__ src, int scols, int srows, uint16_t* __restrict__ dst) {
  const int x = blockIdx.x * blockDim.x + threadIdx.x, y = blockIdx.y * blockDim.y + threadIdx.y;
  if (x >= scols / 2 || y >= srows / 2) return;
  pyr_down_u16_px(src, scols, srows, dst, x, y);
}

__device__ __forceinline__ bool vmap_point(int d, int u, int v, float fx_inv, float fy_inv, float cx, float cy, float cutoff, f3& p) {
  const float z = d / 1000.f;
  if (z != 0 && z < cutoff) {
    p = {z * (u - cx) * fx_inv, z * (v - cy) * fy_inv, z};
    return true;
  }
  return false;
}
__global__ void k_create_vmap(const uint16_t* __restrict__ depth, int cols, int rows, float fx_inv, float fy_inv, float cx,
                              float cy, float cutoff, float* __restrict__ vmap) {
  const int u = blockIdx.x * blockDim.x + threadIdx.x, v = blockIdx.y * blockDim.y + threadIdx.y;
  if (u >= cols || v >= rows) return;
  f3 p;
  if (vmap_point(depth[v * cols + u], u, v, fx_inv, fy_inv, cx, cy, cutoff, p)) {
    vmap[v * cols + u] = p.x;
    vmap[(v + rows) * cols + u] = p.y;
    vmap[(v + 2 * rows) * cols + u] = p.z;
  } else {
    vmap[v * cols + u] = qnan();
  }
}
__global__ void k_create_nmap(const float* __restrict__ vmap, int cols, int rows, float* __restrict__ nmap) {
  const int u = blockIdx.x * blockDim.x + threadIdx.x, v = blockIdx.y * blockDim.y + threadIdx.y;
  if (u >= cols || v >= rows) return;
  if (u == cols - 1 || v == rows - 1) { nmap[v * cols + u] = qnan(); return; }
  const float x00 = vmap[v * cols + u], x01 = vmap[v * cols + u + 1], x10 = vmap[(v + 1) * cols + u];
  if (!isnan(x00) && !isnan(x01) && !isnan(x10)) {
    const f3 v00{x00, vmap[(v + rows) * cols + u], vmap[(v + 2 * rows) * cols + u]};
    const f3 v01{x01, vmap[(v + rows) * cols + u + 1], vmap[(v + 2 * rows) * cols + u + 1]};
    const f3 v10{x10, vmap[(v + 1 + rows) * cols + u], vmap[(v + 1 + 2 * rows) * cols + u]};
    const f3 r = normalized(cross(v01 - v00, v10 - v00));
    nmap[v * cols + u] = r.x;
    nmap[(v + rows) * cols + u] = r.y;
    nmap[(v + 2 * rows) * cols + u] = r.z;
  } else {
    nmap[v * cols + u] = qnan();
  }
}

struct VNLevels {
  const uint16_t* depth[NUM_PYRS];
  float* vmap[NUM_PYRS];
  float* nmap[NUM_PYRS];
  int cols[NUM_PYRS], rows[NUM_PYRS];
  Intr k[NUM_PYRS];
  float cutoff;
};
__device__ __forceinline__ void vmap_nmap_px(const VNLevels& L, int l, int u, int v) {
  const int cols = L.cols[l], rows = L.rows[l];
  if (u >= cols || v >= rows) return;
  const uint16_t* __restrict__ depth = L.depth[l];
  float* __restrict__ vmap = L.vmap[l];
  float* __restrict__ nmap = L.nmap[l];
  const float fx_inv = 1.f / L.k[l].fx, fy_inv = 1.f / L.k[l].fy, cx = L.k[l].cx, cy = L.k[l].cy;
  f3 v00, v01, v10;
  const bool ok00 = vmap_point(depth[v * cols + u], u, v, fx_inv, fy_inv, cx, cy, L.cutoff, v00);
  if (ok00) {
    vmap[v * cols + u] = v00.x;
    vmap[(v + rows) * cols + u] = v00.y;
    vmap[(v + 2 * rows) * cols + u] = v00.z;
  } else {
    vmap[v * cols + u] = qnan();
  }
  if (u == cols - 1 || v == rows - 1) { nmap[v * cols + u] = qnan(); return; }
  const bool ok01 = vmap_point(depth[v * cols + u + 1], u + 1, v, fx_inv, fy_inv, cx, cy, L.cutoff, v01);
  const bool ok10 = vmap_point(depth[(v + 1) * cols + u], u, v + 1, fx_inv, fy_inv, cx, cy, L.cutoff, v10);
  if (ok00 && ok01 && ok10) {
    const f3 r = normalized(cross(v01 - v00, v10 - v00));
    nmap[v * cols + u] = r.x;
    nmap[(v + rows) * cols + u] = r.y;
    nmap[(v + 2 * rows) * cols + u] = r.z;
  } else {
    nmap[v * cols + u] = qnan();
  }
}
__global__ void k_vmap_nmap_levels(const VNLevels L) {
  vmap_nmap_px(L, blockIdx.z, blockIdx.x * blockDim.x + threadIdx.x, blockIdx.y * blockDim.y + threadIdx.y);
}

__global__ void k_transform_maps(const float* __restrict__ vsrc, const float* __restrict__ nsrc, int cols, int rows,
                                 const float* __restrict__ Rp, const float* __restrict__ tp, float* vdst, float* ndst) {
  const int x = blockIdx.x * blockDim.x + threadIdx.x, y = blockIdx.y * blockDim.y + threadIdx.y;
  if (x >= cols || y >= rows) return;
  const m33 R = m33_load(Rp);
  const f3 t{tp[0], tp[1], tp[2]};
  float ox = qnan();
  const float vx = vsrc[y * cols + x];
  if (!isnan(vx)) {
    const f3 vs{vx, vsrc[(y + rows) * cols + x], vsrc[(y + 2 * rows) * cols + x]};
    const f3 vd = mul(R, vs) + t;
    vdst[(y + rows) * cols + x] = vd.y;
    vdst[(y + 2 * rows) * cols + x] = vd.z;
    ox = vd.x;
  }
  vdst[y * cols + x] = ox;
  float onx = qnan();
  const float nx = nsrc[y * cols + x];
  if (!isnan(nx)) {
    const f3 ns{nx, nsrc[(y + rows) * cols + x], nsrc[(y + 2 * rows) * cols + x]};
    const f3 nd = mul(R, ns);
    ndst[(y + rows) * cols + x] = nd.y;
    ndst[(y + 2 * rows) * cols + x] = nd.z;
    onx = nd.x;
  }
  ndst[y * cols + x] = onx;
}

__global__ void k_copy_maps(const float4* __restrict__ vtex, const float4* __restrict__ ntex, int cols, int rows,
                            float4* __restrict__ vmaps_tmp, float* __restrict__ vmap, float* __restrict__ nmap) {
  const int x = blockIdx.x * blockDim.x + threadIdx.x, y = blockIdx.y * blockDim.y + threadIdx.y;
  if (x >= cols || y >= rows) return;
  const float4 vs = vtex[y * cols + x];
  const float4 ns = ntex[y * cols + x];
  vmaps_tmp[y * cols + x] = vs;
  f3 vd{qnan(), qnan(), qnan()}, nd{qnan(), qnan(), qnan()};
  if (!(vs.z == 0)) {
    vd = {vs.x, vs.y, vs.z};
    nd = {ns.x, ns.y, ns.z};
  }
  vmap[y * cols + x] = vd.x;
  vmap[(y + rows) * cols + x] = vd.y;
  vmap[(y + 2 * rows) * cols + x] = vd.z;
  nmap[y * cols + x] = nd.x;
  nmap[(y + rows) * cols + x] = nd.y;
  nmap[(y + 2 * rows) * cols + x] = nd.z;
}

template <bool NORMALIZE>
__global__ void k_resize_map(const float* __restrict__ in, int scols, int srows, float* __restrict__ out) {
  const int dcols = scols / 2, drows = srows / 2;
  const int x = blockIdx.x * blockDim.x + threadIdx.x, y = blockIdx.y * blockDim.y + threadIdx.y;
  if (x >= dcols || y >= drows) return;
  const int xs = x * 2, ys = y * 2;
  const float x00 = in[ys * scols + xs], x01 = in[ys * scols + xs + 1], x10 = in[(ys + 1) * scols + xs], x11 = in[(ys + 1) * scols + xs + 1];
  if (isnan(x00) || isnan(x01) || isnan(x10) || isnan(x11)) { out[y * dcols + x] = qnan(); return; }
  f3 n;
  n.x = (x00 + x01 + x10 + x11) / 4;
  const float* py = in + (size_t)srows * scols;
  const float* pz = in + (size_t)2 * srows * scols;
  n.y = (py[ys * scols + xs] + py[ys * scols + xs + 1] + py[(ys + 1) * scols + xs] + py[(ys + 1) * scols + xs + 1]) / 4;
  n.z = (pz[ys * scols + xs] + pz[ys * scols + xs + 1] + pz[(ys + 1) * scols + xs] + pz[(ys + 1) * scols + xs + 1]) / 4;
  if (NORMALIZE) n = normalized(n);
  out[y * dcols + x] = n.x;
  out[(y + drows) * dcols + x] = n.y;
  out[(y + 2 * drows) * dcols + x] = n.z;
}

__device__ __forceinline__ float gauss25(int idx) {
  const int r = idx / 5, c = idx - r * 5;
  const float wr = r == 2 ? 6.f : ((r == 1 || r == 3) ? 4.f : 1.f);
  const float wc = c == 2 ? 6.f : ((c == 1 || c == 3) ? 4.f : 1.f);
  return wr * wc;
}

__device__ __forceinline__ float gauss5(int r) { return r == 2 ? 6.f : ((r == 1 || r == 3) ? 4.f : 1.f); }
__device__ __forceinline__ void pyr_down_gauss_f_px(const float* __restrict__ src, int scols, int srows, float* __restrict__ dst, int x, int y) {
  const int dcols = scols / 2, D = 5;
  const int tx = min(2 * x - D / 2 + D, scols - 1), ty = min(2 * y - D / 2 + D, srows - 1);
  float vals[D * D];
#pragma unroll
  for (int oy = 0; oy < D; ++oy)
#pragma unroll
    for (int ox = 0; ox < D; ++ox)
      vals[oy * D + ox] = src[min(max(2 * y - D / 2 + oy, 0), srows - 1) * scols + min(max(2 * x - D / 2 + ox, 0), scols - 1)];
  float sum = 0;
  int count = 0;
#pragma unroll
  for (int oy = 0; oy < D; ++oy)
#pragma unroll
    for (int ox = 0; ox < D; ++ox) {
      const int cy = 2 * y - D / 2 + oy, cx = 2 * x - D / 2 + ox;
      const float s = vals[oy * D + ox];
      if (cy >= 0 && cy < ty && cx >= 0 && cx < tx && !isnan(s)) {
        const float g = gauss5(ty - cy - 1) * gauss5(tx - cx - 1);
        sum += s * g;
        count = (int)((float)count + g);
      }
    }
  dst[y * dcols + x] = (float)(sum / (float)count);
}
__global__ void k_pyr_down_gauss_f(const float* __restrict__ src, int scols, int srows, float* __restrict__ dst) {
  const int x = blockIdx.x * blockDim.x + threadIdx.x, y = blockIdx.y * blockDim.y + threadIdx.y;
  if (x >= scols / 2 || y >= srows / 2) return;
  pyr_down_gauss_f_px(src, scols, srows, dst, x, y);
}

__device__ __forceinline__ void pyr_down_uchar_gauss_px(const uint8_t* __restrict__ src, int scols, int srows, uint8_t* __restrict__ dst, int x, int y) {
  const int dcols = scols / 2, D = 5;
  const int tx = min(2 * x - D / 2 + D, scols - 1), ty = min(2 * y - D / 2 + D, srows - 1);
  int vals[D * D];
#pragma unroll
  for (int oy = 0; oy < D; ++oy)
#pragma unroll
    for (int ox = 0; ox < D; ++ox)
      vals[oy * D + ox] = src[min(max(2 * y - D / 2 + oy, 0), srows - 1) * scols + min(max(2 * x - D / 2 + ox, 0), scols - 1)];
  float sum = 0;
  int count = 0;
#pragma unroll
  for (int oy = 0; oy < D; ++oy)
#pragma unroll
    for (int ox = 0; ox < D; ++ox) {
      const int cy = 2 * y - D / 2 + oy, cx = 2 * x - D / 2 + ox;
      const int sv = vals[oy * D + ox];
      if (cy >= 0 && cy < ty && cx >= 0 && cx < tx && sv > 0) {
        const float g = gauss5(ty - cy - 1) * gauss5(tx - cx - 1);
        sum += (float)sv * g;
        count = (int)((float)count + g);
      }
    }
  const float q = sum / (float)count;
  const int iv = (q != q) ? 0 : (int)fminf(fmaxf(q, 0.0f), 255.0f);
  dst[y * dcols + x] = (uint8_t)iv;
}
__global__ void k_pyr_down_uchar_gauss(const uint8_t* __restrict__ src, int scols, int srows, uint8_t* __restrict__ dst) {
  const int x = blockIdx.x * blockDim.x + threadIdx.x, y = blockIdx.y * blockDim.y + threadIdx.y;
  if (x >= scols / 2 || y >= srows / 2) return;
  pyr_down_uchar_gauss_px(src, scols, srows, dst, x, y);
}
struct PyrJobs {
  const void* src[4];
  void* dst[4];
  int type[4];
  int scols, srows;
};
__global__ void k_pyr_down_multi(const PyrJobs J) {
  const int x = blockIdx.x * blockDim.x + threadIdx.x, y = blockIdx.y * blockDim.y + threadIdx.y;
  if (x >= J.scols / 2 || y >= J.srows / 2) return;
  const int j = blockIdx.z;
  if (J.type[j] == 0) pyr_down_u16_px((const uint16_t*)J.src[j], J.scols, J.srows, (uint16_t*)J.dst[j], x, y);
  else if (J.type[j] == 1) pyr_down_gauss_f_px((const float*)J.src[j], J.scols, J.srows, (float*)J.dst[j], x, y);
  else pyr_down_uchar_gauss_px((const uint8_t*)J.src[j], J.scols, J.srows, (uint8_t*)J.dst[j], x, y);
}
__global__ void k_vertices_to_depth(const float4* __restrict__ vmaps_tmp, int cols, int rows, float cutOff, float* __restrict__ dst) {
  const int x = blockIdx.x * blockDim.x + threadIdx.x, y = blockIdx.y * blockDim.y + threadIdx.y;
  if (x >= cols || y >= rows) return;
  const float z = vmaps_tmp[y * cols + x].z;
  dst[y * cols + x] = (z > cutOff || z <= 0) ? qnan() : z;
}

template <int CH>
__global__ void k_bgr_to_intensity(const uint8_t* __restrict__ src, int n, uint8_t* __restrict__ dst) {
  const int i = blockIdx.x * blockDim.x + threadIdx.x;
  if (i >= n) return;
  const uint8_t* s = src + (size_t)i * CH;
  dst[i] = intensity_of((float)s[0], (float)s[1], (float)s[2]);
}
__device__ __forceinline__ bool use_fill_in(const TrackState* __restrict__ st);
__global__ void k_model_intensity(const uint8_t* __restrict__ pred, const uint8_t* __restrict__ fill, bool force_fill,
                                  const TrackState* __restrict__ st, int n, uint8_t* __restrict__ dst) {
  const int i = blockIdx.x * blockDim.x + threadIdx.x;
  if (i >= n) return;
  const uint8_t* src = (force_fill || use_fill_in(st)) ? fill : pred;
  const uchar4 c = ((const uchar4*)src)[i];
  dst[i] = intensity_of((float)c.x, (float)c.y, (float)c.z);
}
__global__ void k_rgba_intensity_pair(const uint8_t* __restrict__ last_rgba, const uint8_t* __restrict__ next_rgba, int n, uint8_t* __restrict__ last0,
                                      uint8_t* __restrict__ next0) {
  const int i = blockIdx.x * blockDim.x + threadIdx.x;
  if (i >= n) return;
  const uchar4 c = ((const uchar4*)(blockIdx.y == 0 ? last_rgba : next_rgba))[i];
  (blockIdx.y == 0 ? last0 : next0)[i] = intensity_of((float)c.x, (float)c.y, (float)c.z);
}

__device__ __forceinline__ float sobel_gsx(int k) {
  const float a = 0.52201f, b = 0.79451f;
  return k == 8 ? -a : k == 7 ? 0.00000f : k == 6 ? a : k == 5 ? -b : k == 4 ? -0.00000f : k == 3 ? b : k == 2 ? -a : k == 1 ? 0.00000f : a;
}
__device__ __forceinline__ float sobel_gsy(int k) {
  const float a = 0.52201f, b = 0.79451f;
  return k == 8 ? -a : k == 7 ? -b : k == 6 ? -a : (k >= 3) ? 0.00000f : k == 2 ? a : k == 1 ? b : a;
}
__device__ __forceinline__ void sobel_taps(const float (&v)[3][3], int cols, int rows, int x, int y, int16_t& dx, int16_t& dy) {
  const float gsx[9] = {0.52201f, 0.00000f, -0.52201f, 0.79451f, -0.00000f, -0.79451f, 0.52201f, 0.00000f, -0.52201f};
  const float gsy[9] = {0.52201f, 0.79451f, 0.52201f, 0.00000f, 0.00000f, 0.00000f, -0.52201f, -0.79451f, -0.52201f};
  float dxVal = 0, dyVal = 0;
  if (x >= 1 && y >= 1 && x <= cols - 2 && y <= rows - 2) {
    int k = 8;
#pragma unroll
    for (int dj = 0; dj < 3; ++dj)
#pragma unroll
      for (int di = 0; di < 3; ++di) {
        dxVal += v[dj][di] * gsx[k];
        dyVal += v[dj][di] * gsy[k];
        --k;
      }
  } else {
    const int jlo = max(y - 1, 0), ilo = max(x - 1, 0), ni = min(x + 1, cols - 1) - ilo + 1;
#pragma unroll
    for (int dj = 0; dj < 3; ++dj)
#pragma unroll
      for (int di = 0; di < 3; ++di) {
        const int j = y - 1 + dj, i = x - 1 + di;
        if (j >= 0 && j <= rows - 1 && i >= 0 && i <= cols - 1) {
          const int k = 8 - ((j - jlo) * ni + (i - ilo));
          dxVal += v[dj][di] * sobel_gsx(k);
          dyVal += v[dj][di] * sobel_gsy(k);
        }
      }
  }
  dx = (int16_t)(int)dxVal;
  dy = (int16_t)(int)dyVal;
}
__device__ __forceinline__ void sobel_px(const uint8_t* __restrict__ src, int cols, int rows, int x, int y, int16_t* dx, int16_t* dy) {
  float v[3][3];
#pragma unroll
  for (int dj = 0; dj < 3; ++dj)
#pragma unroll
    for (int di = 0; di < 3; ++di) v[dj][di] = (float)src[min(max(y - 1 + dj, 0), rows - 1) * cols + min(max(x - 1 + di, 0), cols - 1)];
  int16_t ox, oy;
  sobel_taps(v, cols, rows, x, y, ox, oy);
  dx[y * cols + x] = ox;
  dy[y * cols + x] = oy;
}
__global__ void k_sobel(const uint8_t* __restrict__ src, int cols, int rows, int16_t* __restrict__ dx, int16_t* __restrict__ dy) {
  const int x = blockIdx.x * blockDim.x + threadIdx.x, y = blockIdx.y * blockDim.y + threadIdx.y;
  if (x >= cols || y >= rows) return;
  sobel_px(src, cols, rows, x, y, dx, dy);
}
__device__ __forceinline__ uint32_t pack_corres(int u0, int v0, int idiff) {
  return 0x80000000u | ((uint32_t)(idiff + 255) << 22) | ((uint32_t)v0 << 11) | (uint32_t)u0;
}
struct SobelLevels {
  const uint8_t* src[NUM_PYRS];
  int16_t* dx[NUM_PYRS];
  int16_t* dy[NUM_PYRS];
  const float* nextDepth[NUM_PYRS];
  uint8_t* mask[NUM_PYRS];
  uint32_t* corres[NUM_PYRS];
  float minScale[NUM_PYRS];
  int cols[NUM_PYRS], rows[NUM_PYRS];
};
__device__ __forceinline__ void sobel_mask_px(const SobelLevels& L, int l, int x, int y) {
  const int cols = L.cols[l], rows = L.rows[l];
  if (x >= cols || y >= rows) return;
  const uint8_t* __restrict__ img = L.src[l];
  const int k = y * cols + x;
  int w[4][4];
#pragma unroll
  for (int a = 0; a < 4; ++a)
#pragma unroll
    for (int b = 0; b < 4; ++b) w[a][b] = img[min(max(y - 2 + a, 0), rows - 1) * cols + min(max(x - 2 + b, 0), cols - 1)];
  const float nd = L.nextDepth[l][k];
  float v[3][3];
#pragma unroll
  for (int dj = 0; dj < 3; ++dj)
#pragma unroll
    for (int di = 0; di < 3; ++di) v[dj][di] = (float)w[dj + 1][di + 1];
  int16_t sx, sy;
  sobel_taps(v, cols, rows, x, y, sx, sy);
  L.dx[l][k] = sx;
  L.dy[l][k] = sy;
  bool ok = (x < cols - 5 && y < rows - 1);
#pragma unroll
  for (int a = 0; a < 4; ++a)
#pragma unroll
    for (int b = 0; b < 4; ++b) {
      const int u = y - 2 + a, vv = x - 2 + b;
      if (u >= 0 && u < rows && vv >= 0 && vv < cols) ok = ok && (w[a][b] > 0);
    }
  if (ok) {
    const int valx = sx, valy = sy;
    const float mTwo = (float)((valx * valx) + (valy * valy));
    ok = mTwo >= L.minScale[l] && !isnan(nd);
  }
  L.mask[l][k] = ok ? 1 : 0;
  L.corres[l][k] = 0u;
}
__global__ void k_sobel_levels(const SobelLevels L) {
  sobel_mask_px(L, blockIdx.z, blockIdx.x * blockDim.x + threadIdx.x, blockIdx.y * blockDim.y + threadIdx.y);
}
__global__ void k_vn_sobel_levels(const VNLevels V, const SobelLevels S) {
  const int z = blockIdx.z, x = blockIdx.x * blockDim.x + threadIdx.x, y = blockIdx.y * blockDim.y + threadIdx.y;
  if (z < NUM_PYRS) vmap_nmap_px(V, z, x, y);
  else sobel_mask_px(S, z - NUM_PYRS, x, y);
}

__device__ __forceinline__ f3 project_point(int x, int y, float z, float invFx, float invFy, float cx, float cy) {
  return {(float)((x - cx) * z * invFx), (float)((y - cy) * z * invFy), z};
}
__global__ void k_project_points(const float* __restrict__ depth, int cols, int rows, float invFx, float invFy, float cx,
                                 float cy, float* __restrict__ cloud) {
  const int x = blockIdx.x * blockDim.x + threadIdx.x, y = blockIdx.y * blockDim.y + threadIdx.y;
  if (x >= cols || y >= rows) return;
  const f3 p = project_point(x, y, depth[y * cols + x], invFx, invFy, cx, cy);
  float* c = cloud + (size_t)(y * cols + x) * 3;
  c[0] = p.x; c[1] = p.y; c[2] = p.z;
}

__device__ __forceinline__ bool use_fill_in(const TrackState* __restrict__ st) {
  return !((float)st->dense_count / (float)st->dense_samples > 0.75f);
}
struct ModelMapsArgs {
  const float4* pred_vertex;
  const float4* pred_normal;
  const float4* fill_vertex;
  const float4* fill_normal;
  float* vmap[NUM_PYRS];
  float* nmap[NUM_PYRS];
  float* depth0;
  int cols, rows;
  float maxDepthRGB;
  bool camera_frame;
  const uint8_t* pred_image;
  const uint8_t* fill_image;
  bool force_fill_image;
  uint8_t* last0;
  const uint8_t* tally_image;
  unsigned* tally_out;
};
__device__ __forceinline__ bool model_maps_use_fill(const ModelMapsArgs& A, const TrackState* __restrict__ st, bool first_wg) {
  if (!A.tally_image) return use_fill_in(st);
  __shared__ unsigned tally_s[4];
  const int t = (int)(threadIdx.y * blockDim.x + threadIdx.x);
  const int dc = A.cols / 20, dr = A.rows / 20;
  unsigned cnt = 0;
  for (int i = t; i < dc * dr; i += 256) {
    const int b = i / dc, a = i - b * dc;
    const uchar4 px = ((const uchar4*)A.tally_image)[(20 * b + 10) * A.cols + (20 * a + 10)];
    cnt += (px.x > 0 && px.y > 0 && px.z > 0) ? 1u : 0u;
  }
#pragma unroll
  for (int off = 32; off > 0; off >>= 1) cnt += __shfl_down(cnt, off, 64);
  if ((t & 63) == 0) tally_s[t >> 6] = cnt;
  __syncthreads();
  const unsigned total = tally_s[0] + tally_s[1] + tally_s[2] + tally_s[3];
  if (first_wg && t == 0) *A.tally_out = total;
  return !((float)total / (float)st->dense_samples > 0.75f);
}
template <bool ALL_PLANES>
__device__ __forceinline__ void store_planar(float* m, int cols, int rows, int x, int y, bool valid, f3 v) {
  if (valid) {
    m[(y + rows) * cols + x] = v.y;
    m[(y + 2 * rows) * cols + x] = v.z;
    m[y * cols + x] = v.x;
  } else {
    m[y * cols + x] = qnan();
    if (ALL_PLANES) {
      m[(y + rows) * cols + x] = qnan();
      m[(y + 2 * rows) * cols + x] = qnan();
    }
  }
}
__device__ __forceinline__ float qx1(float x) { return __int_as_float(__builtin_amdgcn_mov_dpp(__float_as_int(x), 0xB1, 0xF, 0xF, true)); }
__device__ __forceinline__ float qx2(float x) { return __int_as_float(__builtin_amdgcn_mov_dpp(__float_as_int(x), 0x4E, 0xF, 0xF, true)); }
__device__ __forceinline__ f3 qx1(f3 v) { return f3{qx1(v.x), qx1(v.y), qx1(v.z)}; }
__device__ __forceinline__ f3 qx2(f3 v) { return f3{qx2(v.x), qx2(v.y), qx2(v.z)}; }
__device__ __forceinline__ f3 box4(f3 a, f3 b, f3 c, f3 d) {
  return f3{(a.x + b.x + c.x + d.x) / 4, (a.y + b.y + c.y + d.y) / 4, (a.z + b.z + c.z + d.z) / 4};
}
__device__ __forceinline__ void model_maps_lane(const ModelMapsArgs& A, const TrackState* __restrict__ st, int gx, int by, bool fill) {
  const int cols = A.cols, rows = A.rows;
  if (gx >= cols || by * 4 >= rows) return;
  const int j = gx & 3, bx = gx >> 2;
  const bool even = (j & 1) == 0, leftpair = j < 2;
  const float4* __restrict__ vsrc = fill ? A.fill_vertex : A.pred_vertex;
  const float4* __restrict__ nsrc = fill ? A.fill_normal : A.pred_normal;
  const m33 R = m33_load(st->R_wc_f);
  const f3 t{st->t_wc_f[0], st->t_wc_f[1], st->t_wc_f[2]};
  const bool cf = A.camera_frame;
  const int c1 = cols / 2, r1 = rows / 2, c2 = cols / 4, r2 = rows / 4;
  float4 vs[4], ns[4];
#pragma unroll
  for (int r = 0; r < 4; ++r) {
    vs[r] = vsrc[(by * 4 + r) * cols + gx];
    ns[r] = nsrc[(by * 4 + r) * cols + gx];
  }
  if (A.last0) {
    const uchar4* __restrict__ isrc = (const uchar4*)((A.force_fill_image || fill) ? A.fill_image : A.pred_image);
    uchar4 cs[4];
#pragma unroll
    for (int r = 0; r < 4; ++r) cs[r] = isrc[(by * 4 + r) * cols + gx];
#pragma unroll
    for (int r = 0; r < 4; ++r) A.last0[(by * 4 + r) * cols + gx] = intensity_of((float)cs[r].x, (float)cs[r].y, (float)cs[r].z);
  }
  f3 v0[4], n0[4];
#pragma unroll
  for (int r = 0; r < 4; ++r) {
    const int y = by * 4 + r;
    const bool ok = !(vs[r].z == 0);
    v0[r] = {vs[r].x, vs[r].y, vs[r].z};
    n0[r] = {ns[r].x, ns[r].y, ns[r].z};
    A.depth0[y * cols + gx] = (vs[r].z > A.maxDepthRGB || vs[r].z <= 0) ? qnan() : vs[r].z;
    const bool nok = ok && !isnan(ns[r].x);
    if (cf) {
      store_planar<true>(A.vmap[0], cols, rows, gx, y, ok, v0[r]);
      store_planar<true>(A.nmap[0], cols, rows, gx, y, ok, n0[r]);
    } else {
      store_planar<true>(A.vmap[0], cols, rows, gx, y, ok && !isnan(vs[r].x), mul(R, v0[r]) + t);
      store_planar<true>(A.nmap[0], cols, rows, gx, y, nok, mul(R, n0[r]));
    }
  }
  f3 v1[2], n1[2];
  bool v1ok[2], n1ok[2];
#pragma unroll
  for (int qy = 0; qy < 2; ++qy) {
    const f3 pv0 = qx1(v0[2 * qy]), pv1 = qx1(v0[2 * qy + 1]), pn0 = qx1(n0[2 * qy]), pn1 = qx1(n0[2 * qy + 1]);
    const f3 va = even ? v0[2 * qy] : pv0, vb = even ? pv0 : v0[2 * qy], vc = even ? v0[2 * qy + 1] : pv1, vd = even ? pv1 : v0[2 * qy + 1];
    const f3 na_ = even ? n0[2 * qy] : pn0, nb = even ? pn0 : n0[2 * qy], nc = even ? n0[2 * qy + 1] : pn1, nd = even ? pn1 : n0[2 * qy + 1];
    const bool oka = !(va.z == 0), okb = !(vb.z == 0), okc = !(vc.z == 0), okd = !(vd.z == 0);
    const bool vok = oka && okb && okc && okd && !isnan(va.x) && !isnan(vb.x) && !isnan(vc.x) && !isnan(vd.x);
    const bool nok = oka && okb && okc && okd && !isnan(na_.x) && !isnan(nb.x) && !isnan(nc.x) && !isnan(nd.x);
    const f3 vavg = box4(va, vb, vc, vd);
    const f3 navg = normalized(box4(na_, nb, nc, nd));
    v1[qy] = vavg; n1[qy] = navg;
    v1ok[qy] = vok; n1ok[qy] = nok;
    if (even) {
      const int x1 = bx * 2 + (j >> 1), y1 = by * 2 + qy;
      if (cf) {
        store_planar<false>(A.vmap[1], c1, r1, x1, y1, vok, vavg);
        store_planar<false>(A.nmap[1], c1, r1, x1, y1, nok, navg);
      } else {
        store_planar<false>(A.vmap[1], c1, r1, x1, y1, vok && !isnan(vavg.x), mul(R, vavg) + t);
        store_planar<false>(A.nmap[1], c1, r1, x1, y1, nok && !isnan(navg.x), mul(R, navg));
      }
    }
  }
  const f3 ov0 = qx2(v1[0]), ov1 = qx2(v1[1]), on0 = qx2(n1[0]), on1 = qx2(n1[1]);
  const bool ovok0 = qx2(v1ok[0] ? 1.0f : 0.0f) != 0.0f, ovok1 = qx2(v1ok[1] ? 1.0f : 0.0f) != 0.0f;
  const bool onok0 = qx2(n1ok[0] ? 1.0f : 0.0f) != 0.0f, onok1 = qx2(n1ok[1] ? 1.0f : 0.0f) != 0.0f;
  const f3 v00 = leftpair ? v1[0] : ov0, v01 = leftpair ? ov0 : v1[0], v10 = leftpair ? v1[1] : ov1, v11 = leftpair ? ov1 : v1[1];
  const f3 n00 = leftpair ? n1[0] : on0, n01 = leftpair ? on0 : n1[0], n10 = leftpair ? n1[1] : on1, n11 = leftpair ? on1 : n1[1];
  const bool vok2 = v1ok[0] && ovok0 && v1ok[1] && ovok1 && !isnan(v00.x) && !isnan(v01.x) && !isnan(v10.x) && !isnan(v11.x);
  const bool nok2 = n1ok[0] && onok0 && n1ok[1] && onok1 && !isnan(n00.x) && !isnan(n01.x) && !isnan(n10.x) && !isnan(n11.x);
  const f3 va = box4(v00, v01, v10, v11);
  const f3 na = normalized(box4(n00, n01, n10, n11));
  if (j == 0) {
    if (cf) {
      store_planar<false>(A.vmap[2], c2, r2, bx, by, vok2, va);
      store_planar<false>(A.nmap[2], c2, r2, bx, by, nok2, na);
    } else {
      store_planar<false>(A.vmap[2], c2, r2, bx, by, vok2 && !isnan(va.x), mul(R, va) + t);
      store_planar<false>(A.nmap[2], c2, r2, bx, by, nok2 && !isnan(na.x), mul(R, na));
    }
  }
}
__global__ void __launch_bounds__(256) k_model_maps(const ModelMapsArgs A, const TrackState* __restrict__ st) {
  const bool fill = model_maps_use_fill(A, st, blockIdx.x == 0 && blockIdx.y == 0);
  model_maps_lane(A, st, (int)(blockIdx.x * blockDim.x + threadIdx.x), (int)(blockIdx.y * blockDim.y + threadIdx.y), fill);
}
struct IcpView {
  const float* vmap_curr;
  const float* nmap_curr;
  const float* vmap_g_prev;
  const float* nmap_g_prev;
  int cols, rows;
  Intr k;
  float distThres, angleThres;
  float dist2Max, sine2Max;
};
struct IcpPose { m33 Rcurr; f3 tcurr; m33 Rprev_inv; f3 tprev; };
__device__ __forceinline__ float uniform_f(float x) { return __uint_as_float(__builtin_amdgcn_readfirstlane(__float_as_uint(x))); }
__device__ __forceinline__ f3 uniform_f3(f3 a) { return f3{uniform_f(a.x), uniform_f(a.y), uniform_f(a.z)}; }
__device__ __forceinline__ m33 uniform_m33(const m33& m) { return m33{{uniform_f3(m.r[0]), uniform_f3(m.r[1]), uniform_f3(m.r[2])}}; }
__device__ __forceinline__ IcpPose icp_pose_uniform(const IcpPose& P) {
  return IcpPose{uniform_m33(P.Rcurr), uniform_f3(P.tcurr), uniform_m33(P.Rprev_inv), uniform_f3(P.tprev)};
}

__device__ __forceinline__ bool icp_row(const IcpView& V, const IcpPose& P, int x, int y, float (&row)[7]) {
  const int cols = V.cols, rows = V.rows;
  const int plane = cols * rows, idx = y * cols + x;
  const f3 vcurr{V.vmap_curr[idx], V.vmap_curr[idx + plane], V.vmap_curr[idx + 2 * plane]};
  const f3 vcurr_g = mul(P.Rcurr, vcurr) + P.tcurr;
  const f3 vcurr_cp = mul(P.Rprev_inv, vcurr_g - P.tprev);
  const int ux = f2i_rn(vcurr_cp.x * V.k.fx / vcurr_cp.z + V.k.cx);
  const int uy = f2i_rn(vcurr_cp.y * V.k.fy / vcurr_cp.z + V.k.cy);
  if (ux < 0 || uy < 0 || ux >= cols || uy >= rows || vcurr_cp.z < 0) return false;
  const int pidx = uy * cols + ux;
  const f3 vprev_g{V.vmap_g_prev[pidx], V.vmap_g_prev[pidx + plane], V.vmap_g_prev[pidx + 2 * plane]};
  const f3 ncurr{V.nmap_curr[idx], V.nmap_curr[idx + plane], V.nmap_curr[idx + 2 * plane]};
  const f3 ncurr_g = mul(P.Rcurr, ncurr);
  const f3 nprev_g{V.nmap_g_prev[pidx], V.nmap_g_prev[pidx + plane], V.nmap_g_prev[pidx + 2 * plane]};
  const float dist = norm(vprev_g - vcurr_g);
  const float sine = norm(cross(ncurr_g, nprev_g));
  if (!(sine < V.angleThres && dist <= V.distThres && !isnan(ncurr.x) && !isnan(nprev_g.x))) return false;
  const f3 s_cp = mul(P.Rprev_inv, vcurr_g - P.tprev);
  const f3 d_cp = mul(P.Rprev_inv, vprev_g - P.tprev);
  const f3 n_cp = mul(P.Rprev_inv, nprev_g);
  const f3 c = cross(s_cp, n_cp);
  row[0] = n_cp.x; row[1] = n_cp.y; row[2] = n_cp.z;
  row[3] = c.x; row[4] = c.y; row[5] = c.z;
  row[6] = dot(n_cp, s_cp - d_cp);
  return true;
}

struct RgbView {
  const void* corres;
  const float* lastDepth;
  const float* cloud;
  const int16_t* dIdx;
  const int16_t* dIdy;
  int cols, rows;
  Intr k;
  float sobelScale;
};
template <bool PACKED>
__device__ __forceinline__ bool rgb_row(const RgbView& V, float sigma, int i, float (&row)[7]) {
  int zx, zy, oi;
  float diff;
  if (PACKED) {
    const uint32_t c = ((const uint32_t*)V.corres)[i];
    if (!(c & 0x80000000u)) return false;
    zx = (int)(c & 0x7FFu); zy = (int)((c >> 11) & 0x7FFu);
    diff = (float)((int)((c >> 22) & 0x1FFu) - 255);
    oi = i;
  } else {
    const DataTerm c = ((const DataTerm*)V.corres)[i];
    if (!c.valid) return false;
    zx = c.zero_x; zy = c.zero_y;
    diff = c.diff;
    oi = c.one_y * V.cols + c.one_x;
  }
  float w = sigma + fabsf(diff);
  w = w > 1.19209290E-07F ? 1.0f / w : 1.0f;
  if (sigma == -1) w = 1;
  row[6] = -w * diff;
  f3 p;
  const int zi = zy * V.cols + zx;
  if (V.cloud) {
    p = {V.cloud[(size_t)zi * 3], V.cloud[(size_t)zi * 3 + 1], V.cloud[(size_t)zi * 3 + 2]};
  } else {
    p = project_point(zx, zy, V.lastDepth[zi], 1.0f / V.k.fx, 1.0f / V.k.fy, V.k.cx, V.k.cy);
  }
  const float invz = (float)(1.0 / (double)p.z);
  const float dI_dx_val = w * V.sobelScale * V.dIdx[oi];
  const float dI_dy_val = w * V.sobelScale * V.dIdy[oi];
  const float v0 = dI_dx_val * V.k.fx * invz;
  const float v1 = dI_dy_val * V.k.fy * invz;
  const float v2 = -(v0 * p.x + v1 * p.y) * invz;
  row[0] = v0; row[1] = v1; row[2] = v2;
  row[3] = -p.z * v1 + p.y * v2;
  row[4] = p.z * v0 - p.x * v2;
  row[5] = -p.y * v0 + p.x * v1;
  return true;
}

struct ResidualView {
  const int16_t* dIdx;
  const int16_t* dIdy;
  const float* lastDepth;
  const float* nextDepth;
  const uint8_t* lastImage;
  const uint8_t* nextImage;
  DataTerm* corres;
  int cols, rows;
  float minScale, maxDepthDelta;
};
__device__ __forceinline__ void residual_px(const ResidualView& V, const m33& K, const f3& kt, int k, int& cnt, int& sq) {
  const int cols = V.cols, rows = V.rows;
  const int i = k / cols, j0 = k - i * cols;
  DataTerm corres;
  corres.zero_x = corres.zero_y = corres.one_x = corres.one_y = 0;
  corres.diff = 0.f;
  corres.valid = 0;
  corres.pad[0] = corres.pad[1] = corres.pad[2] = 0;
  if (j0 < cols - 5 && i < rows - 1) {
    bool valid = true;
    for (int u = max(i - 2, 0); u < min(i + 2, rows); ++u)
      for (int v = max(j0 - 2, 0); v < min(j0 + 2, cols); ++v) valid = valid && (V.nextImage[u * cols + v] > 0);
    if (valid) {
      const int valx = V.dIdx[k], valy = V.dIdy[k];
      const float mTwo = (float)((valx * valx) + (valy * valy));
      if (mTwo >= V.minScale) {
        const int y = i, x = j0;
        const float d1 = V.nextDepth[k];
        if (!isnan(d1)) {
          const float transformed_d1 = (float)(d1 * (K.r[2].x * x + K.r[2].y * y + K.r[2].z) + kt.z);
          const int u0 = f2i_rn((d1 * (K.r[0].x * x + K.r[0].y * y + K.r[0].z) + kt.x) / transformed_d1);
          const int v0 = f2i_rn((d1 * (K.r[1].x * x + K.r[1].y * y + K.r[1].z) + kt.y) / transformed_d1);
          if (u0 >= 0 && v0 >= 0 && u0 < cols && v0 < rows) {
            const float d0 = V.lastDepth[v0 * cols + u0];
            const uint8_t li = V.lastImage[v0 * cols + u0];
            if (d0 > 0 && fabsf(transformed_d1 - d0) <= V.maxDepthDelta && li != 0) {
              corres.zero_x = (short)u0; corres.zero_y = (short)v0;
              corres.one_x = (short)x; corres.one_y = (short)y;
              corres.diff = (float)V.nextImage[k] - (float)li;
              corres.valid = 1;
              cnt += 1;
// ... 1932 lines not shown
```

### include/ef_hip.h

```cpp
#ifndef EF_HIP_H_
#define EF_HIP_H_
#include <stddef.h>
#include <stdint.h>
#ifdef __cplusplus
extern "C" {
#endif

#define EF_OK 0
#define EF_EINVAL (-1)
#define EF_EHIP (-2)
#define EF_ENOMEM (-3)
#define EF_ESTATE (-4)
#define EF_ECAPACITY (-5)

typedef struct ef_ctx ef_ctx;

typedef struct ef_config {
  int width, height;
  float fx, fy, cx, cy;
  int time_delta;
  float confidence;
  float depth_cut;
  float icp_weight;
  int fast_odom;
// ... 171 lines not shown
  int color_type;
  int draw_window;
  int time;
  int time_delta;
} ef_render_params;
int ef_default_render_params(ef_ctx* ctx, ef_render_params* params);
int ef_render_model(ef_ctx* ctx, const ef_render_params* params, uint8_t* rgba, float* depth, float* vertex, float* normal,
                    uint32_t* index);
int ef_render_model_dev(ef_ctx* ctx, const ef_render_params* params, uint8_t* rgba_dev, float* depth_dev, float* vertex_dev,
                        float* normal_dev, uint32_t* index_dev);

int ef_set_surfel_ids(ef_ctx* ctx, int on);
int ef_get_surfel_ids(ef_ctx* ctx, uint32_t* ids, uint32_t max_ids, uint32_t* count);
int ef_enable_labels(ef_ctx* ctx, int num_classes);
int ef_set_labels(ef_ctx* ctx, const float* probs, uint32_t count);
int ef_get_labels(ef_ctx* ctx, uint32_t* ids_or_null, float* probs_or_null, uint32_t max_rows, uint32_t* count);
int ef_fuse_labels(ef_ctx* ctx, const ef_render_params* view_or_null, const float* probs_chw);
int ef_fuse_labels_dev(ef_ctx* ctx, const ef_render_params* view_or_null, const float* probs_chw_dev);
int ef_render_labels(ef_ctx* ctx, const ef_render_params* params, int32_t* label, float* prob);
int ef_render_labels_dev(ef_ctx* ctx, const ef_render_params* params, int32_t* label_dev, float* prob_dev);

#define EF_QUERY_MAX_RATIO 16
#define EF_QUERY_DEFAULT_CELL 0.02f
int ef_set_query_cell(ef_ctx* ctx, float cell_m);
int ef_query_nearest(ef_ctx* ctx, const float* points3, uint32_t n, float max_dist, float min_conf, uint32_t* row, uint32_t* id_or_null,
                     float* dist2_or_null, float* plane_or_null);
int ef_query_knn(ef_ctx* ctx, const float* points3, uint32_t n, int k, float max_dist, float min_conf, uint32_t* rows, float* dist2_or_null,
                 uint32_t* count_or_null);
int ef_query_nearest_dev(ef_ctx* ctx, const float* points3_dev, uint32_t n, float max_dist, float min_conf, uint32_t* row_dev,
                         uint32_t* id_dev_or_null, float* dist2_dev_or_null, float* plane_dev_or_null);
int ef_query_knn_dev(ef_ctx* ctx, const float* points3_dev, uint32_t n, int k, float max_dist, float min_conf, uint32_t* rows_dev,
                     float* dist2_dev_or_null, uint32_t* count_dev_or_null);

#define EF_REGISTER_MAX_ITERATIONS 100
#define EF_REGISTER_SMALL_ANGLE 1e-4
#define EF_REG_CONVERGED 0
#define EF_REG_MAX_ITERATIONS 1
#define EF_REG_TOO_FEW_PAIRS 2
#define EF_REG_DEGENERATE 3
typedef struct ef_register_params {
  float max_dist;
  float min_conf;
  float min_normal_cos;
  int max_iterations;
  int min_pairs;
  double stop_translation;
  double stop_rotation;
} ef_register_params;
typedef struct ef_register_sums {
  double A[36];
  double b[6];
  double e;
  uint32_t pairs;
  uint32_t points;
} ef_register_sums;
typedef struct ef_register_result {
  int status;
  int iterations;
  uint32_t pairs;
  double rms_first;
  double rms_last;
  double A[36];
} ef_register_result;
int ef_default_register_params(ef_ctx* ctx, ef_register_params* params);
int ef_register_step(ef_ctx* ctx, const float* points3, const float* normals3_or_null, uint32_t n, const ef_register_params* params,
                     const double* T16_or_null, ef_register_sums* out, uint32_t* row_or_null, float* plane_or_null);
int ef_register_update(const ef_register_sums* sums, const double* T16_or_null, double* T16_out, double* xi6_or_null);
int ef_register_cloud(ef_ctx* ctx, const float* points3, const float* normals3_or_null, uint32_t n, const ef_register_params* params,
                      const double* T_init16_or_null, double* T_out16, ef_register_result* result, uint32_t* row_or_null,
                      float* plane_or_null);
int ef_register_step_dev(ef_ctx* ctx, const float* points3_dev, const float* normals3_dev_or_null, uint32_t n,
                         const ef_register_params* params, const double* T16_or_null, ef_register_sums* out, uint32_t* row_dev_or_null,
                         float* plane_dev_or_null);
int ef_register_cloud_dev(ef_ctx* ctx, const float* points3_dev, const float* normals3_dev_or_null, uint32_t n,
                          const ef_register_params* params, const double* T_init16_or_null, double* T_out16, ef_register_result* result,
                          uint32_t* row_dev_or_null, float* plane_dev_or_null);

#define EF_SEL_BOX        0x01u
#define EF_SEL_CONF       0x02u
#define EF_SEL_INIT_TIME  0x04u
#define EF_SEL_LAST_TIME  0x08u
#define EF_SEL_RADIUS     0x10u
#define EF_SEL_ID         0x20u
#define EF_SEL_LABEL      0x40u
#define EF_SEL_INVERT     0x100u
typedef struct ef_map_selection {
  uint32_t tests;
  double T_bw[16];
  float box_min[3], box_max[3];
  float conf_min, conf_max;
  int init_time_min, init_time_max;
  int last_time_min, last_time_max;
  float radius_min, radius_max;
  uint32_t id_min, id_max;
  int label_class;
  float label_min_prob;
} ef_map_selection;
void ef_default_map_selection(ef_map_selection* sel);
int ef_map_select(ef_ctx* ctx, const ef_map_selection* sel, uint32_t* rows, uint32_t max_rows, uint32_t* count);
int ef_map_select_dev(ef_ctx* ctx, const ef_map_selection* sel, uint32_t* rows_dev, uint32_t max_rows, uint32_t* count_dev);
int ef_map_gather(ef_ctx* ctx, const uint32_t* rows, uint32_t n, float* surfels12);
int ef_map_gather_dev(ef_ctx* ctx, const uint32_t* rows_dev, uint32_t n, float* surfels12_dev);
int ef_map_erase(ef_ctx* ctx, const ef_map_selection* sel, uint32_t* removed_or_null);
int ef_map_erase_rows(ef_ctx* ctx, const uint32_t* rows, uint32_t n, uint32_t* removed_or_null);
int ef_map_erase_rows_dev(ef_ctx* ctx, const uint32_t* rows_dev, uint32_t n, uint32_t* removed_or_null);

#define EF_INSERT_KEEP (-1)
#define EF_INSERT_MAX_RECORDS 0x0FFFFFFFu
typedef struct ef_insert_params {
  int   gate;
  float min_separation;
  float min_conf;
  float min_normal_cos;
  int   init_time;
  int   last_time;
} ef_insert_params;
typedef struct ef_insert_result { uint32_t inserted, duplicates, skipped, count_after; } ef_insert_result;
int ef_default_insert_params(ef_ctx* ctx, ef_insert_params* params);
int ef_map_insert(ef_ctx* ctx, const float* surfels12, uint32_t n, const double* T16_or_null, const ef_insert_params* params,
                  ef_insert_result* result, uint32_t* new_row_or_null, uint32_t* match_row_or_null);
int ef_map_insert_dev(ef_ctx* ctx, const float* surfels12_dev, uint32_t n, const double* T16_or_null, const ef_insert_params* params,
                      ef_insert_result* result, uint32_t* new_row_dev_or_null, uint32_t* match_row_dev_or_null);

#define EF_FUSE_SKIPPED    0
#define EF_FUSE_NOVEL      1
#define EF_FUSE_WEIGHTLESS 2
#define EF_FUSE_ABSORBED   3
#define EF_FUSE_FUSED      4
#define EF_FUSE_INSERTED   5
typedef struct ef_fuse_params {
  float min_separation, min_conf, min_normal_cos;
  int   append;
  int   init_time;
  int   last_time;
} ef_fuse_params;
typedef struct ef_fuse_result { uint32_t fused, absorbed, weightless, novel, skipped, inserted, count_after; } ef_fuse_result;
int ef_default_fuse_params(ef_ctx* ctx, ef_fuse_params* params);
int ef_map_fuse(ef_ctx* ctx, const float* surfels12, uint32_t n, const double* T16_or_null, const ef_fuse_params* params, ef_fuse_result* result,
                uint32_t* new_row_or_null, uint32_t* match_row_or_null, uint8_t* outcome_or_null);
int ef_map_fuse_dev(ef_ctx* ctx, const float* surfels12_dev, uint32_t n, const double* T16_or_null, const ef_fuse_params* params,
                    ef_fuse_result* result, uint32_t* new_row_dev_or_null, uint32_t* match_row_dev_or_null, uint8_t* outcome_dev_or_null);

#define EF_THIN_KEEP_MAX_CONF 0
#define EF_THIN_KEEP_NEWEST   1
#define EF_THIN_KEEP_FIRST    2
#define EF_THIN_ROWS_REMOVED         0
#define EF_THIN_ROWS_REPRESENTATIVES 1
typedef struct ef_thin_params { float cell; int keep; } ef_thin_params;
typedef struct ef_thin_result { uint32_t participants, cells, removed, count_after; } ef_thin_result;
int ef_default_thin_params(ef_ctx* ctx, ef_thin_params* params);
int ef_map_thin_select(ef_ctx* ctx, const ef_thin_params* params, const ef_map_selection* among_or_null, int what, uint32_t* rows,
                       uint32_t max_rows, uint32_t* count);
int ef_map_thin_select_dev(ef_ctx* ctx, const ef_thin_params* params, const ef_map_selection* among_or_null, int what, uint32_t* rows_dev,
                           uint32_t max_rows, uint32_t* count_dev);
int ef_map_thin(ef_ctx* ctx, const ef_thin_params* params, const ef_map_selection* among_or_null, ef_thin_result* result);

#define EF_CARVE_MAX_VIEWS 32
typedef struct ef_carve_params {
  int   width, height;
  float fx, fy, cx, cy;
  float min_depth, max_depth;
  float margin, margin_quad;
  int   window;
  int   min_views;
  int   protect;
} ef_carve_params;
typedef struct ef_carve_views {
  int n;
  const double* T_wc16;
  const uint16_t* depth;
} ef_carve_views;
typedef struct ef_carve_result { uint32_t participants, observed, free_space, protected_, removed, count_after; } ef_carve_result;
int ef_default_carve_params(ef_ctx* ctx, ef_carve_params* params);
int ef_map_carve_select(ef_ctx* ctx, const ef_carve_params* params, const ef_carve_views* views, const ef_map_selection* among_or_null,
                        uint32_t* rows, uint32_t max_rows, uint32_t* count, uint8_t* votes2_or_null);
int ef_map_carve_select_dev(ef_ctx* ctx, const ef_carve_params* params, const ef_carve_views* views_depth_dev,
                            const ef_map_selection* among_or_null, uint32_t* rows_dev, uint32_t max_rows, uint32_t* count_dev,
                            uint8_t* votes2_dev_or_null);
int ef_map_carve(ef_ctx* ctx, const ef_carve_params* params, const ef_carve_views* views, const ef_map_selection* among_or_null,
                 ef_carve_result* result);
int ef_map_carve_dev(ef_ctx* ctx, const ef_carve_params* params, const ef_carve_views* views_depth_dev, const ef_map_selection* among_or_null,
                     ef_carve_result* result);

enum ef_image {
  EF_IMG_DEPTH_FILTERED = 0,
  EF_IMG_DEPTH_METRIC,
  EF_IMG_DEPTH_METRIC_FILTERED,
  EF_IMG_PREDICT_IMAGE,
  EF_IMG_PREDICT_VERTEX,
  EF_IMG_PREDICT_NORMAL,
  EF_IMG_PREDICT_TIME,
  EF_IMG_FILL_IMAGE,
  EF_IMG_FILL_VERTEX,
  EF_IMG_FILL_NORMAL,
  EF_IMG_INDEX,
  EF_IMG_VERT_CONF,
  EF_IMG_COLOR_TIME,
  EF_IMG_NORM_RAD,
  EF_IMG_OLD_IMAGE,
  EF_IMG_OLD_VERTEX,
  EF_IMG_OLD_NORMAL,
  EF_IMG_OLD_TIME
};
int ef_get_image(ef_ctx* ctx, int which, void* host_dst, size_t bytes);
int ef_get_image_resized(ef_ctx* ctx, int which, int factor, void* host_dst, size_t bytes);
int ef_get_tracker_buffer(ef_ctx* ctx, int which, int level, void* host_dst, size_t bytes);
int ef_get_tracker_buffer_of(ef_ctx* ctx, int tracker, int which, int level, void* host_dst, size_t bytes);

typedef struct ef_timing { const char* name; float ms; } ef_timing;
int ef_enable_timing(ef_ctx* ctx, int on);
int ef_get_timings(ef_ctx* ctx, ef_timing* out, int max, int* n);

typedef struct ef_kernel_time {
  const char* name; float avg_us; int launches; double bytes_per_launch; double bytes_per_launch_survey;
} ef_kernel_time;
int ef_kernel_timing(ef_ctx* ctx, int every_n_frames);
int ef_get_kernel_timing(ef_ctx* ctx, ef_kernel_time* out);
int ef_get_splat_timing(ef_ctx* ctx, ef_kernel_time* out);
int ef_get_tracker_timing(ef_ctx* ctx, ef_kernel_time* out);

int ef_get_tracker_fallbacks(ef_ctx* ctx, int* count);
typedef struct ef_tracker_plan {
  int script, n_small, n_iter;
  unsigned long long levels;
  unsigned res_bytes, res_budget;
} ef_tracker_plan;
int ef_get_tracker_plan(ef_ctx* ctx, ef_tracker_plan* out);
int ef_debug_occupy(ef_ctx* ctx, int workgroups, int microseconds);
int ef_debug_query_lanes(ef_ctx* ctx, int lanes);
int ef_debug_inject_tracker_abort(ef_ctx* ctx);

int ef_debug_clocks(ef_ctx* ctx, unsigned long long* out16);
int ef_debug_small_clocks(ef_ctx* ctx, unsigned long long* out32);

int ef_dev_alloc(void** dev, size_t bytes);
int ef_dev_free(void* dev);
int ef_dev_upload(void* dev, const void* host, size_t bytes);
int ef_dev_download(void* host, const void* dev, size_t bytes);
int ef_dev_memset(void* dev, int value, size_t bytes);
int ef_dev_sync(void);
int ef_dev_calibrate(void* stream, float* empty_us, float* stream16mb_us);
int ef_device_count(int* n);
int ef_set_device(int device);

typedef struct ef_intr { float fx, fy, cx, cy; } ef_intr;

int ef_op_pyr_down(const uint16_t* src, int src_cols, int src_rows, uint16_t* dst, void* stream);
int ef_op_create_vmap(const ef_intr* intr, const uint16_t* depth, int cols, int rows, float depth_cutoff,
                      float* vmap, void* stream);
int ef_op_create_nmap(const float* vmap, int cols, int rows, float* nmap, void* stream);
int ef_op_transform_maps(const float* vmap_src, const float* nmap_src, int cols, int rows, const float* R9,
                         const float* t3, float* vmap_dst, float* nmap_dst, void* stream);
int ef_op_copy_maps(const float* vmap_src_f4, const float* nmap_src_f4, int cols, int rows, float* vmaps_tmp,
                    float* vmap_dst, float* nmap_dst, void* stream);
int ef_op_resize_vmap(const float* in, int src_cols, int src_rows, float* out, void* stream);
int ef_op_resize_nmap(const float* in, int src_cols, int src_rows, float* out, void* stream);
int ef_op_pyr_down_gauss_f(const float* src, int src_cols, int src_rows, float* dst, void* stream);
int ef_op_pyr_down_uchar_gauss(const uint8_t* src, int src_cols, int src_rows, uint8_t* dst, void* stream);
int ef_op_vertices_to_depth(const float* vmaps_tmp, int cols, int rows, float cutoff, float* dst, void* stream);
int ef_op_image_bgr_to_intensity(const uint8_t* rgba, int cols, int rows, uint8_t* dst, void* stream);
int ef_op_compute_derivative_images(const uint8_t* src, int cols, int rows, int16_t* dx, int16_t* dy, void* stream);
int ef_op_project_to_point_cloud(const float* depth, int cols, int rows, const ef_intr* intr_level0, int level,
                                 float* cloud_f3, void* stream);
int ef_op_icp_step(const float* Rcurr9, const float* tcurr3, const float* vmap_curr, const float* nmap_curr,
                   const float* Rprev_inv9, const float* tprev3, const ef_intr* intr, const float* vmap_g_prev,
                   const float* nmap_g_prev, float dist_thres, float angle_thres, int cols, int rows,
                   float* A_host36, float* b_host6, float* residual_host2, void* stream);
int ef_op_compute_rgb_residual(float min_scale, const int16_t* dIdx, const int16_t* dIdy, const float* last_depth,
                               const float* next_depth, const uint8_t* last_image, const uint8_t* next_image,
                               void* corres_img, float max_depth_delta, const float* kt3, const float* krkinv9,
                               int cols, int rows, int* sigma_sum_host, int* count_host, void* stream);
int ef_op_rgb_step(const void* corres_img, float sigma, const float* cloud_f3, float fx, float fy,
                   const int16_t* dIdx, const int16_t* dIdy, float sobel_scale, int cols, int rows,
                   float* A_host36, float* b_host6, void* stream);
int ef_op_so3_step(const uint8_t* last_image, const uint8_t* next_image, const float* image_basis9,
                   const float* kinv9, const float* krlr9, int cols, int rows, float* A_host9, float* b_host3,
                   float* residual_host2, void* stream);

typedef struct ef_model_maps_op {
  int cols, rows;
  const float *pred_vertex, *pred_normal, *fill_vertex, *fill_normal;
  const uint8_t *pred_image, *fill_image;
  float R[9], t[3];
  float max_depth_rgb;
  int camera_frame, force_fill_image, tally;
  unsigned dense_count;
  int dense_samples;
  float* vmap[3];
  float* nmap[3];
  float* depth0;
  uint8_t* last0;
  int joint;
  const uint16_t* raw;
  const uint8_t* rgb3;
  float depth_cut;
  uint16_t* filtered;
  float* metric;
  float* metric_filtered;
  uint8_t* next0;
} ef_model_maps_op;
int ef_op_model_maps(const ef_model_maps_op* args, unsigned* dense_count_left, void* stream);
int ef_op_sobel_mask(const uint8_t* const* next_image3, const float* const* next_depth3, int cols, int rows, int16_t* const* dIdx3,
                     int16_t* const* dIdy3, uint8_t* const* mask3, uint32_t* const* corres3, void* stream);

enum ef_linalg_op {
  EF_LINALG_LDLT6 = 0,
  EF_LINALG_LDLT3F,
  EF_LINALG_POLAR3,
  EF_LINALG_RODRIGUES,
  EF_LINALG_SE3_INVERSE,
  EF_LINALG_SE3_LOG_NORM,
  EF_LINALG_SCALAR,
  EF_LINALG_LDLT6_WAVE,
  EF_LINALG_LDLT6_EVERY_LANE,
  EF_LINALG_MAT_TO_QUAT,
  EF_LINALG_SE3_MUL,
  EF_LINALG_SE3_CASTF,
  EF_LINALG_SE3_INVERSE_F,
  EF_LINALG_M4_AFFINE_INVERSE,
  EF_LINALG_LDLT_PIVOTS,
  EF_LINALG_LU_INVERSE6
};
int ef_op_linalg(int which, const double* in_host, int n_in, double* out_host, int n_out);

typedef struct ef_gn_state {
  float Rcurr[9], tcurr[3];
  double resultRt[16];
  float krkinv[9], kt[3];
  float lastRGBErrorLevel;
  int rgb_broken;
} ef_gn_state;
typedef struct ef_gn_update_args {
  float sums[58];
  ef_gn_state prev;
  float Rprev[9], tprev[3];
  int count, sigma;
  int icp, rgb, rgb_only;
  float icp_weight;
  ef_intr knext;
  int level_changes;
  int split_tail;
} ef_gn_update_args;
int ef_op_gn_update(const ef_gn_update_args* in, ef_gn_state* next, double* lastA36, double* lastb6, float* stats4);
typedef struct ef_track_end_out {
  double q[4], t[3];
  double logged[16];
  float T_cw[16], pose_f[16], R_wc_f[9], t_wc_f[3];
  float weighting;
} ef_track_end_out;
int ef_op_track_end_tail(const float* Rcurr9, const float* tcurr3, const float* Rprev9, const float* tprev3, const double* q_prev4,
                         const double* t_prev3, int rgb, float weight_multiplier, ef_track_end_out* out);

typedef struct ef_cam { int cols, rows; float fx, fy, cx, cy; } ef_cam;

int ef_op_filter_depth(const uint16_t* raw, int cols, int rows, float max_d, uint16_t* filtered, void* stream);
int ef_op_metricise_depth(const uint16_t* in, int cols, int rows, float max_d, float* out, void* stream);
int ef_op_seed_map(const ef_cam* cam, const uint8_t* rgb, const float* depth_metric, const float* depth_metric_filtered,
                   int time, float max_depth, float* surfels_aos, uint32_t* count_host, void* stream);
int ef_op_predict_indices(const ef_cam* cam, const double* T_wc16, int time, const float* surfels_aos, uint32_t count,
                          float max_depth, int time_delta, uint32_t* index_map, float* vert_conf, float* color_time,
                          float* norm_rad, void* stream);
int ef_op_combined_predict(const ef_cam* cam, const double* T_wc16, const float* surfels_aos, uint32_t count,
                           float max_depth, float conf_threshold, int time, int max_time, int time_delta,
                           uint8_t* image_rgba, float* vertex, float* normal, uint16_t* time_map, void* stream);
int ef_op_synthesize_depth(const ef_cam* cam, const double* T_wc16, const float* surfels_aos, uint32_t count,
                           float max_depth, float conf_threshold, int time, int max_time, int time_delta,
                           float* depth, void* stream);
int ef_op_fill_in(const ef_cam* cam, const uint8_t* image_rgba, const float* vertex, const float* normal,
                  const uint16_t* depth_filtered, const uint8_t* rgb, int passthrough, int passthrough_image,
                  uint8_t* fill_image, float* fill_vertex, float* fill_normal, void* stream);
int ef_op_dense_enough(const ef_cam* cam, const uint8_t* image_rgba, int* dense_host, void* stream);
int ef_op_fuse(const ef_cam* cam, const double* T_wc16, int time, const uint8_t* rgb, const float* depth_metric,
               const float* depth_metric_filtered, const uint32_t* index_map, const float* vert_conf,
               const float* color_time, const float* norm_rad, float max_depth, float weighting, float* surfels_aos,
               uint32_t count, float* new_unstable_aos, uint32_t* new_count_host, void* stream);
int ef_op_clean(const ef_cam* cam, const double* T_wc16, int time, const uint32_t* index_map, const float* vert_conf,
                const float* color_time, const float* norm_rad, float conf_threshold, int time_delta, float max_depth,
                const float* surfels_aos, uint32_t count, const float* new_unstable_aos, uint32_t new_count,
                float* surfels_out_aos, uint32_t* out_count_host, void* stream);
int ef_op_clean_deform(const ef_cam* cam, const double* T_wc16, int time, const uint32_t* index_map, const float* vert_conf,
                       const float* color_time, const float* norm_rad, float conf_threshold, int time_delta, float max_depth,
                       const float* surfels_aos, uint32_t count, const float* new_unstable_aos, uint32_t new_count,
                       const float* graph, int nodes, const float* depth, int is_fern, float* surfels_out_aos,
                       uint32_t* out_count_host, void* stream);

#ifdef __cplusplus
}
#endif
#endif
```

Baseline: 2176.

## Fuse pyramid build into two staged kernels with shared-memory level-2 tiles

Replaces the per-level pyramid downsampling launches and the combined vmap/nmap/sobel launch with two kernels. Stage A does the level-0 maps, level-0 sobel and the level-0-to-1 downsampling in one flat grid. Stage B computes the level-2 downsampled depth and image into shared-memory tiles and derives level-2 vmap/nmap and sobel from them directly, recomputing halo pixels rather than rereading global memory. It also makes the filter inner loops branch-free with selects and adds a Python/C test entry point. This removes several launches and inter-level dependencies, at the cost of redundant halo computation and more complex block-index dispatch.

New measurement: 2172. About the same (-0.2%).

```diff
diff --git a/elasticfusion_amd/api.py b/elasticfusion_amd/api.py
--- a/elasticfusion_amd/api.py
+++ b/elasticfusion_amd/api.py
@@ -1473,6 +1473,24 @@
         return tuple([b.to_array(dt, (h >> l, w >> l)) for l, b in enumerate(bufs)] for bufs, dt in zip(outs, (np.int16, np.int16, np.uint8, np.uint32)))
 
     @staticmethod
+    def build_pyramids(depth_filtered, lastDepth0, lastImage0, nextImage0, intr, cutoff, with_sobel=True):
+        h, w = depth_filtered.shape
+        kinds = dict(depth_tmp=(np.uint16, 1), lastDepth=(np.float32, 1), lastImage=(np.uint8, 1), nextImage=(np.uint8, 1), vmap_curr=(np.float32, 3),
+                     nmap_curr=(np.float32, 3), dIdx=(np.int16, 1), dIdy=(np.int16, 1), mask=(np.uint8, 1), corres=(np.uint32, 1))
+        level0 = dict(depth_tmp=depth_filtered, lastDepth=lastDepth0, lastImage=lastImage0, nextImage=nextImage0)
+        bufs = {}
+        for name, (dt, planes) in kinds.items():
+            bufs[name] = [DevBuf(planes * (h >> l) * (w >> l) * np.dtype(dt).itemsize, fill=0xA5) for l in range(3)]
+            if name in level0:
+                assert level0[name].shape == (h, w), (name, level0[name].shape)
+                bufs[name][0] = DevBuf.from_array(np.ascontiguousarray(level0[name], dt))
+        arr = lambda name: (P * 3)(*[b.p for b in bufs[name]])
+        k = ef_intr(*[float(v) for v in intr])
+        _chk(lib().ef_op_build_pyramids(arr("depth_tmp"), arr("lastDepth"), arr("lastImage"), arr("nextImage"), w, h, C.byref(k), float(cutoff),
+                                        int(with_sobel), arr("vmap_curr"), arr("nmap_curr"), arr("dIdx"), arr("dIdy"), arr("mask"), arr("corres"), None))
+        return {name: [b.to_array(dt, (planes * (h >> l), w >> l)) for l, b in enumerate(bufs[name])] for name, (dt, planes) in kinds.items()}
+
+    @staticmethod
     def clean_deform(cam, T_wc, time, idx, vc, ct, nr, confThreshold, timeDelta, maxDepth, surfels, newUnstable, graph, depth, isFern=0):
         s = ops._f32(surfels).reshape(-1, 12)
         nu = ops._f32(newUnstable).reshape(-1, 12)
diff --git a/elasticfusion_amd/csrc/ef_host_ops.inc b/elasticfusion_amd/csrc/ef_host_ops.inc
--- a/elasticfusion_amd/csrc/ef_host_ops.inc
+++ b/elasticfusion_amd/csrc/ef_host_ops.inc
@@ -219,6 +219,26 @@
     o.nextImage[i] = nextImage[i]; o.nextDepth[i] = nextDepth[i]; o.dIdx[i] = dIdx[i]; o.dIdy[i] = dIdy[i]; o.mask[i] = mask[i]; o.corres[i] = corres[i];
   }
   eft::sobel_mask_op(o, (hipStream_t)s);
+  const hipError_t le = hipGetLastError();
+  if (le != hipSuccess) { g_create_error = hipGetErrorString(le); return EF_EHIP; }
+  OP_SYNC(s);
+  return EF_OK;
+}
+int ef_op_build_pyramids(uint16_t* const* depth, float* const* lastDepth, uint8_t* const* lastImage, uint8_t* const* nextImage, int cols, int rows,
+                         const ef_intr* k, float cutoff, int with_sobel, float* const* vmap, float* const* nmap, int16_t* const* dIdx,
+                         int16_t* const* dIdy, uint8_t* const* mask, uint32_t* const* corres, void* s) {
+  if (!depth || !lastDepth || !lastImage || !nextImage || !k || !vmap || !nmap || !dIdx || !dIdy || !mask || !corres) return EF_EINVAL;
+  if (cols < 4 || rows < 4 || cols > 2048 || rows > 2048) return EF_EINVAL;
+  eft::BuildPyramidsOp o{};
+  o.cols = cols; o.rows = rows;
+  o.k = eft::Intr{k->fx, k->fy, k->cx, k->cy};
+  o.cutoff = cutoff; o.with_sobel = with_sobel != 0;
+  for (int i = 0; i < eft::NUM_PYRS; ++i) {
+    if (!depth[i] || !lastDepth[i] || !lastImage[i] || !nextImage[i] || !vmap[i] || !nmap[i] || !dIdx[i] || !dIdy[i] || !mask[i] || !corres[i]) return EF_EINVAL;
+    o.depth[i] = depth[i]; o.lastDepth[i] = lastDepth[i]; o.lastImage[i] = lastImage[i]; o.nextImage[i] = nextImage[i];
+    o.vmap[i] = vmap[i]; o.nmap[i] = nmap[i]; o.dIdx[i] = dIdx[i]; o.dIdy[i] = dIdy[i]; o.mask[i] = mask[i]; o.corres[i] = corres[i];
+  }
+  eft::build_pyramids_op(o, (hipStream_t)s);
   const hipError_t le = hipGetLastError();
   if (le != hipSuccess) { g_create_error = hipGetErrorString(le); return EF_EHIP; }
   OP_SYNC(s);
diff --git a/elasticfusion_amd/csrc/ef_track.hpp b/elasticfusion_amd/csrc/ef_track.hpp
--- a/elasticfusion_amd/csrc/ef_track.hpp
+++ b/elasticfusion_amd/csrc/ef_track.hpp
@@ -216,6 +216,23 @@
   uint32_t* corres[NUM_PYRS];
 };
 void sobel_mask_op(const SobelMaskOp& o, hipStream_t s);
+struct BuildPyramidsOp {
+  int cols, rows;
+  Intr k;
+  float cutoff;
+  bool with_sobel;
+  uint16_t* depth[NUM_PYRS];
+  float* lastDepth[NUM_PYRS];
+  uint8_t* lastImage[NUM_PYRS];
+  uint8_t* nextImage[NUM_PYRS];
+  float* vmap[NUM_PYRS];
+  float* nmap[NUM_PYRS];
+  int16_t* dIdx[NUM_PYRS];
+  int16_t* dIdy[NUM_PYRS];
+  uint8_t* mask[NUM_PYRS];
+  uint32_t* corres[NUM_PYRS];
+};
+void build_pyramids_op(const BuildPyramidsOp& o, hipStream_t s);
 void init_first_rgb(const Pyramid& p, const uint8_t* rgb3, hipStream_t s);
 struct TrackTail {
   int cur, slots;
diff --git a/elasticfusion_amd/csrc/ef_track_host_inputs.inc b/elasticfusion_amd/csrc/ef_track_host_inputs.inc
--- a/elasticfusion_amd/csrc/ef_track_host_inputs.inc
+++ b/elasticfusion_amd/csrc/ef_track_host_inputs.inc
@@ -18,14 +18,17 @@
 }
 struct PyrJob { const void* src; void* dst; int type; };
 enum { PYR_U16 = 0, PYR_F32 = 1, PYR_U8 = 2 };
-void launch_pyr_step(const Pyramid& p, int i, std::initializer_list<PyrJob> jobs, hipStream_t s) {
+PyrJobs pyr_jobs_of(const Pyramid& p, int i, std::initializer_list<PyrJob> jobs) {
   PyrJobs J{};
   int n = 0;
   for (const PyrJob& j : jobs) { J.src[n] = j.src; J.dst[n] = j.dst; J.type[n] = j.type; ++n; }
   J.scols = p.W(i); J.srows = p.H(i);
+  return J;
+}
+void launch_pyr_step(const Pyramid& p, int i, std::initializer_list<PyrJob> jobs, hipStream_t s) {
   dim3 g = tile_grid(p.W(i + 1), p.H(i + 1));
-  g.z = n;
-  hipLaunchKernelGGL(k_pyr_down_multi, g, tile_block(), 0, s, J);
+  g.z = (unsigned)jobs.size();
+  hipLaunchKernelGGL(k_pyr_down_multi, g, tile_block(), 0, s, pyr_jobs_of(p, i, jobs));
 }
 inline const uint16_t* frame_depth(const Pyramid& p, const uint16_t* depth_filtered, int i) { return i == 0 ? depth_filtered : p.depth_tmp[i]; }
 
@@ -41,7 +44,7 @@
   }
   return L;
 }
-void build_vn_levels(const Pyramid& p, const uint16_t* depth_filtered, Intr k, float cutoff, bool with_sobel, hipStream_t s) {
+VNLevels vn_levels_of(const Pyramid& p, const uint16_t* depth_filtered, Intr k, float cutoff) {
   VNLevels L;
   for (int i = 0; i < NUM_PYRS; ++i) {
     L.depth[i] = frame_depth(p, depth_filtered, i);
@@ -52,14 +55,12 @@
     L.k[i] = intr_level(k, i);
   }
   L.cutoff = cutoff;
+  return L;
+}
+void build_vn_levels(const Pyramid& p, const uint16_t* depth_filtered, Intr k, float cutoff, hipStream_t s) {
   dim3 g = tile_grid(p.W(0), p.H(0));
-  if (with_sobel) {
-    g.z = 2 * NUM_PYRS;
-    hipLaunchKernelGGL(k_vn_sobel_levels, g, tile_block(), 0, s, L, sobel_levels_of(p));
-    return;
-  }
   g.z = NUM_PYRS;
-  hipLaunchKernelGGL(k_vmap_nmap_levels, g, tile_block(), 0, s, L);
+  hipLaunchKernelGGL(k_vmap_nmap_levels, g, tile_block(), 0, s, vn_levels_of(p, depth_filtered, k, cutoff));
 }
 ModelMapsArgs model_maps_choice_args(const Pyramid& p, bool model_side, const float* pred_vertex, const float* pred_normal, const float* fill_vertex,
                                      const float* fill_normal, const TrackState* st, float maxDepthRGB, const uint8_t* pred_image_rgba,
@@ -143,15 +144,38 @@
                            {p.lastImage[i], p.lastImage[i + 1], PYR_U8}, {p.nextImage[i], p.nextImage[i + 1], PYR_U8}}, s);
 }
 void build_pyramids(const Pyramid& p, const uint16_t* depth_filtered, Intr k, float cutoff, hipStream_t s, bool with_sobel) {
-  for (int i = 0; i + 1 < NUM_PYRS; ++i)
-    launch_pyr_step(p, i, {{frame_depth(p, depth_filtered, i), p.depth_tmp[i + 1], PYR_U16}, {p.lastDepth[i], p.lastDepth[i + 1], PYR_F32},
-                           {p.lastImage[i], p.lastImage[i + 1], PYR_U8}, {p.nextImage[i], p.nextImage[i + 1], PYR_U8}}, s);
-  build_vn_levels(p, depth_filtered, k, cutoff, with_sobel, s);
+  const VNLevels V = vn_levels_of(p, depth_filtered, k, cutoff);
+  const SobelLevels S = sobel_levels_of(p);
+  const dim3 g0 = tile_grid(p.W(0), p.H(0)), g1 = tile_grid(p.W(1), p.H(1));
+  const int n0 = (int)(g0.x * g0.y), n1 = (int)(g1.x * g1.y);
+  const PyrJobs J = pyr_jobs_of(p, 0, {{depth_filtered, p.depth_tmp[1], PYR_U16}, {p.lastDepth[0], p.lastDepth[1], PYR_F32},
+                                       {p.lastImage[0], p.lastImage[1], PYR_U8}, {p.nextImage[0], p.nextImage[1], PYR_U8}});
+  const PyrStageA A{(int)g0.x, n0, with_sobel ? n0 : 0, (int)g1.x, n1};
+  hipLaunchKernelGGL(k_pyr_stage_a, dim3(A.n_maps + A.n_sobel + 4 * A.n_pyr), tile_block(), 0, s, V, S, J, A);
+  PyrStageB B{};
+  B.tiles_x = ceil_div(p.W(2), L2_TW); B.n_tiles = B.tiles_x * ceil_div(p.H(2), L2_TH);
+  B.l1_gx = (int)g1.x; B.n_maps = n1; B.n_sobel = with_sobel ? n1 : 0;
+  B.with_sobel = with_sobel;
+  B.depth1 = p.depth_tmp[1]; B.depth2 = p.depth_tmp[2];
+  B.lastDepth1 = p.lastDepth[1]; B.lastDepth2 = p.lastDepth[2];
+  B.lastImage1 = p.lastImage[1]; B.lastImage2 = p.lastImage[2];
+  B.nextImage1 = p.nextImage[1]; B.nextImage2 = p.nextImage[2];
+  hipLaunchKernelGGL(k_pyr_stage_b, dim3(2 * B.n_tiles + B.n_maps + B.n_sobel), tile_block(), 0, s, V, S, B);
+}
+void build_pyramids_op(const BuildPyramidsOp& o, hipStream_t s) {
+  Pyramid p{};
+  p.width = o.cols; p.height = o.rows;
+  for (int i = 0; i < NUM_PYRS; ++i) {
+    p.depth_tmp[i] = o.depth[i]; p.lastDepth[i] = p.nextDepth[i] = o.lastDepth[i]; p.lastImage[i] = o.lastImage[i]; p.nextImage[i] = o.nextImage[i];
+    p.vmap_curr[i] = o.vmap[i]; p.nmap_curr[i] = o.nmap[i];
+    p.dIdx[i] = o.dIdx[i]; p.dIdy[i] = o.dIdy[i]; p.rgbMask[i] = o.mask[i]; p.corres[i] = o.corres[i];
+  }
+  build_pyramids(p, o.depth[0], o.k, o.cutoff, s, o.with_sobel);
 }
 void build_pyramids_frame_side(const Pyramid& p, const uint16_t* depth_filtered, Intr k, float cutoff, hipStream_t s) {
   for (int i = 0; i + 1 < NUM_PYRS; ++i)
     launch_pyr_step(p, i, {{frame_depth(p, depth_filtered, i), p.depth_tmp[i + 1], PYR_U16}, {p.nextImage[i], p.nextImage[i + 1], PYR_U8}}, s);
-  build_vn_levels(p, depth_filtered, k, cutoff, false, s);
+  build_vn_levels(p, depth_filtered, k, cutoff, s);
 }
 void build_pyramids_model_side(const Pyramid& p, hipStream_t s) {
   for (int i = 0; i + 1 < NUM_PYRS; ++i)
diff --git a/elasticfusion_amd/csrc/ef_track_kernels.hip b/elasticfusion_amd/csrc/ef_track_kernels.hip
--- a/elasticfusion_amd/csrc/ef_track_kernels.hip
+++ b/elasticfusion_amd/csrc/ef_track_kernels.hip
@@ -20,8 +20,7 @@
 inline dim3 tile_block() { return dim3(TILE_X, TILE_Y); }
 
 
-__device__ __forceinline__ void pyr_down_u16_px(const uint16_t* __restrict__ src, int scols, int srows, uint16_t* __restrict__ dst, int x, int y) {
-  const int dcols = scols / 2;
+__device__ __forceinline__ uint16_t pyr_down_u16_val(const uint16_t* __restrict__ src, int scols, int srows, int x, int y) {
   const int D = 5;
   const float sigma_color = 30.f;
   int vals[D * D];
@@ -38,15 +37,18 @@
     for (int xi = -D / 2; xi <= D / 2; ++xi) {
       const bool in = 2 * x + xi >= 0 && 2 * x + xi < scols && 2 * y + yi >= 0 && 2 * y + yi < srows;
       const int val = vals[(yi + D / 2) * D + xi + D / 2];
-      if (in && abs(val - center) < 3 * sigma_color) {
-        const int ax = abs(xi), ay = abs(yi);
-        const float wx = ax == 0 ? 0.375f : (ax == 1 ? 0.25f : 0.0625f);
-        const float wy = ay == 0 ? 0.375f : (ay == 1 ? 0.25f : 0.0625f);
-        sum += (float)val * wx * wy;
-        wall += wx * wy;
-      }
-    }
-  dst[y * dcols + x] = (uint16_t) static_cast<int>(sum / wall);
+      const bool take = in && abs(val - center) < 3 * sigma_color;
+      const int ax = abs(xi), ay = abs(yi);
+      const float wx = ax == 0 ? 0.375f : (ax == 1 ? 0.25f : 0.0625f);
+      const float wy = ay == 0 ? 0.375f : (ay == 1 ? 0.25f : 0.0625f);
+      const float sum1 = sum + (float)val * wx * wy, wall1 = wall + wx * wy;
+      sum = take ? sum1 : sum;
+      wall = take ? wall1 : wall;
+    }
+  return (uint16_t) static_cast<int>(sum / wall);
+}
+__device__ __forceinline__ void pyr_down_u16_px(const uint16_t* __restrict__ src, int scols, int srows, uint16_t* __restrict__ dst, int x, int y) {
+  dst[y * (scols / 2) + x] = pyr_down_u16_val(src, scols, srows, x, y);
 }
 __global__ void k_pyr_down_u16(const uint16_t* __restrict__ src, int scols, int srows, uint16_t* __restrict__ dst) {
   const int x = blockIdx.x * blockDim.x + threadIdx.x, y = blockIdx.y * blockDim.y + threadIdx.y;
@@ -101,15 +103,27 @@
   Intr k[NUM_PYRS];
   float cutoff;
 };
-__device__ __forceinline__ void vmap_nmap_px(const VNLevels& L, int l, int u, int v) {
+template <typename T>
+struct ImageInMemory {
+  const T* __restrict__ p;
+  int stride;
+  __device__ __forceinline__ T at(int x, int y) const { return p[y * stride + x]; }
+};
+template <typename T>
+struct ImageTile {
+  const T* p;
+  int stride, x0, y0;
+  __device__ __forceinline__ T at(int x, int y) const { return p[(y - y0) * stride + (x - x0)]; }
+};
+template <typename Depth>
+__device__ __forceinline__ void vmap_nmap_at(const Depth& depth, const VNLevels& L, int l, int u, int v) {
   const int cols = L.cols[l], rows = L.rows[l];
   if (u >= cols || v >= rows) return;
-  const uint16_t* __restrict__ depth = L.depth[l];
   float* __restrict__ vmap = L.vmap[l];
   float* __restrict__ nmap = L.nmap[l];
   const float fx_inv = 1.f / L.k[l].fx, fy_inv = 1.f / L.k[l].fy, cx = L.k[l].cx, cy = L.k[l].cy;
   f3 v00, v01, v10;
-  const bool ok00 = vmap_point(depth[v * cols + u], u, v, fx_inv, fy_inv, cx, cy, L.cutoff, v00);
+  const bool ok00 = vmap_point(depth.at(u, v), u, v, fx_inv, fy_inv, cx, cy, L.cutoff, v00);
   if (ok00) {
     vmap[v * cols + u] = v00.x;
     vmap[(v + rows) * cols + u] = v00.y;
@@ -118,8 +132,8 @@
     vmap[v * cols + u] = qnan();
   }
   if (u == cols - 1 || v == rows - 1) { nmap[v * cols + u] = qnan(); return; }
-  const bool ok01 = vmap_point(depth[v * cols + u + 1], u + 1, v, fx_inv, fy_inv, cx, cy, L.cutoff, v01);
-  const bool ok10 = vmap_point(depth[(v + 1) * cols + u], u, v + 1, fx_inv, fy_inv, cx, cy, L.cutoff, v10);
+  const bool ok01 = vmap_point(depth.at(u + 1, v), u + 1, v, fx_inv, fy_inv, cx, cy, L.cutoff, v01);
+  const bool ok10 = vmap_point(depth.at(u, v + 1), u, v + 1, fx_inv, fy_inv, cx, cy, L.cutoff, v10);
   if (ok00 && ok01 && ok10) {
     const f3 r = normalized(cross(v01 - v00, v10 - v00));
     nmap[v * cols + u] = r.x;
@@ -128,6 +142,9 @@
   } else {
     nmap[v * cols + u] = qnan();
   }
+}
+__device__ __forceinline__ void vmap_nmap_px(const VNLevels& L, int l, int u, int v) {
+  vmap_nmap_at(ImageInMemory<uint16_t>{L.depth[l], L.cols[l]}, L, l, u, v);
 }
 __global__ void k_vmap_nmap_levels(const VNLevels L) {
   vmap_nmap_px(L, blockIdx.z, blockIdx.x * blockDim.x + threadIdx.x, blockIdx.y * blockDim.y + threadIdx.y);
@@ -209,8 +226,8 @@
 }
 
 __device__ __forceinline__ float gauss5(int r) { return r == 2 ? 6.f : ((r == 1 || r == 3) ? 4.f : 1.f); }
-__device__ __forceinline__ void pyr_down_gauss_f_px(const float* __restrict__ src, int scols, int srows, float* __restrict__ dst, int x, int y) {
-  const int dcols = scols / 2, D = 5;
+__device__ __forceinline__ float pyr_down_gauss_f_val(const float* __restrict__ src, int scols, int srows, int x, int y) {
+  const int D = 5;
   const int tx = min(2 * x - D / 2 + D, scols - 1), ty = min(2 * y - D / 2 + D, srows - 1);
   float vals[D * D];
 #pragma unroll
@@ -218,21 +235,23 @@
 #pragma unroll
     for (int ox = 0; ox < D; ++ox)
       vals[oy * D + ox] = src[min(max(2 * y - D / 2 + oy, 0), srows - 1) * scols + min(max(2 * x - D / 2 + ox, 0), scols - 1)];
-  float sum = 0;
-  int count = 0;
+  float sum = 0, count = 0;
 #pragma unroll
   for (int oy = 0; oy < D; ++oy)
 #pragma unroll
     for (int ox = 0; ox < D; ++ox) {
       const int cy = 2 * y - D / 2 + oy, cx = 2 * x - D / 2 + ox;
       const float s = vals[oy * D + ox];
-      if (cy >= 0 && cy < ty && cx >= 0 && cx < tx && !isnan(s)) {
-        const float g = gauss5(ty - cy - 1) * gauss5(tx - cx - 1);
-        sum += s * g;
-        count = (int)((float)count + g);
-      }
-    }
-  dst[y * dcols + x] = (float)(sum / (float)count);
+      const bool take = cy >= 0 && cy < ty && cx >= 0 && cx < tx && !isnan(s);
+      const float g = gauss5(ty - cy - 1) * gauss5(tx - cx - 1);
+      const float sum1 = sum + s * g, count1 = count + g;
+      sum = take ? sum1 : sum;
+      count = take ? count1 : count;
+    }
+  return (float)(sum / count);
+}
+__device__ __forceinline__ void pyr_down_gauss_f_px(const float* __restrict__ src, int scols, int srows, float* __restrict__ dst, int x, int y) {
+  dst[y * (scols / 2) + x] = pyr_down_gauss_f_val(src, scols, srows, x, y);
 }
 __global__ void k_pyr_down_gauss_f(const float* __restrict__ src, int scols, int srows, float* __restrict__ dst) {
   const int x = blockIdx.x * blockDim.x + threadIdx.x, y = blockIdx.y * blockDim.y + threadIdx.y;
@@ -240,8 +259,8 @@
   pyr_down_gauss_f_px(src, scols, srows, dst, x, y);
 }
 
-__device__ __forceinline__ void pyr_down_uchar_gauss_px(const uint8_t* __restrict__ src, int scols, int srows, uint8_t* __restrict__ dst, int x, int y) {
-  const int dcols = scols / 2, D = 5;
+__device__ __forceinline__ uint8_t pyr_down_uchar_gauss_val(const uint8_t* __restrict__ src, int scols, int srows, int x, int y) {
+  const int D = 5;
   const int tx = min(2 * x - D / 2 + D, scols - 1), ty = min(2 * y - D / 2 + D, srows - 1);
   int vals[D * D];
 #pragma unroll
@@ -249,23 +268,25 @@
 #pragma unroll
     for (int ox = 0; ox < D; ++ox)
       vals[oy * D + ox] = src[min(max(2 * y - D / 2 + oy, 0), srows - 1) * scols + min(max(2 * x - D / 2 + ox, 0), scols - 1)];
-  float sum = 0;
-  int count = 0;
+  float sum = 0, count = 0;
 #pragma unroll
   for (int oy = 0; oy < D; ++oy)
 #pragma unroll
     for (int ox = 0; ox < D; ++ox) {
       const int cy = 2 * y - D / 2 + oy, cx = 2 * x - D / 2 + ox;
       const int sv = vals[oy * D + ox];
-      if (cy >= 0 && cy < ty && cx >= 0 && cx < tx && sv > 0) {
-        const float g = gauss5(ty - cy - 1) * gauss5(tx - cx - 1);
-        sum += (float)sv * g;
-        count = (int)((float)count + g);
-      }
-    }
-  const float q = sum / (float)count;
+      const bool take = cy >= 0 && cy < ty && cx >= 0 && cx < tx && sv > 0;
+      const float g = gauss5(ty - cy - 1) * gauss5(tx - cx - 1);
+      const float sum1 = sum + (float)sv * g, count1 = count + g;
+      sum = take ? sum1 : sum;
+      count = take ? count1 : count;
+    }
+  const float q = sum / count;
   const int iv = (q != q) ? 0 : (int)fminf(fmaxf(q, 0.0f), 255.0f);
-  dst[y * dcols + x] = (uint8_t)iv;
+  return (uint8_t)iv;
+}
+__device__ __forceinline__ void pyr_down_uchar_gauss_px(const uint8_t* __restrict__ src, int scols, int srows, uint8_t* __restrict__ dst, int x, int y) {
+  dst[y * (scols / 2) + x] = pyr_down_uchar_gauss_val(src, scols, srows, x, y);
 }
 __global__ void k_pyr_down_uchar_gauss(const uint8_t* __restrict__ src, int scols, int srows, uint8_t* __restrict__ dst) {
   const int x = blockIdx.x * blockDim.x + threadIdx.x, y = blockIdx.y * blockDim.y + threadIdx.y;
@@ -278,13 +299,14 @@
   int type[4];
   int scols, srows;
 };
-__global__ void k_pyr_down_multi(const PyrJobs J) {
-  const int x = blockIdx.x * blockDim.x + threadIdx.x, y = blockIdx.y * blockDim.y + threadIdx.y;
+__device__ __forceinline__ void pyr_job_px(const PyrJobs& J, int j, int x, int y) {
   if (x >= J.scols / 2 || y >= J.srows / 2) return;
-  const int j = blockIdx.z;
   if (J.type[j] == 0) pyr_down_u16_px((const uint16_t*)J.src[j], J.scols, J.srows, (uint16_t*)J.dst[j], x, y);
   else if (J.type[j] == 1) pyr_down_gauss_f_px((const float*)J.src[j], J.scols, J.srows, (float*)J.dst[j], x, y);
   else pyr_down_uchar_gauss_px((const uint8_t*)J.src[j], J.scols, J.srows, (uint8_t*)J.dst[j], x, y);
+}
+__global__ void k_pyr_down_multi(const PyrJobs J) {
+  pyr_job_px(J, blockIdx.z, blockIdx.x * blockDim.x + threadIdx.x, blockIdx.y * blockDim.y + threadIdx.y);
 }
 __global__ void k_vertices_to_depth(const float4* __restrict__ vmaps_tmp, int cols, int rows, float cutOff, float* __restrict__ dst) {
   const int x = blockIdx.x * blockDim.x + threadIdx.x, y = blockIdx.y * blockDim.y + threadIdx.y;
@@ -319,11 +341,15 @@
 
 __device__ __forceinline__ float sobel_gsx(int k) {
   const float a = 0.52201f, b = 0.79451f;
-  return k == 8 ? -a : k == 7 ? 0.00000f : k == 6 ? a : k == 5 ? -b : k == 4 ? -0.00000f : k == 3 ? b : k == 2 ? -a : k == 1 ? 0.00000f : a;
+  const int r = k / 3, c = k - 3 * r;
+  const float m = r == 1 ? b : a, z = k == 4 ? -0.00000f : 0.00000f;
+  return c == 0 ? m : (c == 2 ? -m : z);
 }
 __device__ __forceinline__ float sobel_gsy(int k) {
   const float a = 0.52201f, b = 0.79451f;
-  return k == 8 ? -a : k == 7 ? -b : k == 6 ? -a : (k >= 3) ? 0.00000f : k == 2 ? a : k == 1 ? b : a;
+  const int r = k / 3, c = k - 3 * r;
+  const float m = c == 1 ? b : a;
+  return r == 0 ? m : (r == 2 ? -m : 0.00000f);
 }
 __device__ __forceinline__ void sobel_taps(const float (&v)[3][3], int cols, int rows, int x, int y, int16_t& dx, int16_t& dy) {
   const float gsx[9] = {0.52201f, 0.00000f, -0.52201f, 0.79451f, -0.00000f, -0.79451f, 0.52201f, 0.00000f, -0.52201f};
@@ -346,11 +372,11 @@
 #pragma unroll
       for (int di = 0; di < 3; ++di) {
         const int j = y - 1 + dj, i = x - 1 + di;
-        if (j >= 0 && j <= rows - 1 && i >= 0 && i <= cols - 1) {
-          const int k = 8 - ((j - jlo) * ni + (i - ilo));
-          dxVal += v[dj][di] * sobel_gsx(k);
-          dyVal += v[dj][di] * sobel_gsy(k);
-        }
+        const bool in = (j >= 0) & (j <= rows - 1) & (i >= 0) & (i <= cols - 1);
+        const int k = 8 - ((j - jlo) * ni + (i - ilo));
+        const float dx1 = dxVal + v[dj][di] * sobel_gsx(k), dy1 = dyVal + v[dj][di] * sobel_gsy(k);
+        dxVal = in ? dx1 : dxVal;
+        dyVal = in ? dy1 : dyVal;
       }
   }
   dx = (int16_t)(int)dxVal;
@@ -385,17 +411,15 @@
   float minScale[NUM_PYRS];
   int cols[NUM_PYRS], rows[NUM_PYRS];
 };
-__device__ __forceinline__ void sobel_mask_px(const SobelLevels& L, int l, int x, int y) {
+template <typename Image>
+__device__ __forceinline__ void sobel_mask_at(const Image& img, float nd, const SobelLevels& L, int l, int x, int y) {
   const int cols = L.cols[l], rows = L.rows[l];
-  if (x >= cols || y >= rows) return;
-  const uint8_t* __restrict__ img = L.src[l];
   const int k = y * cols + x;
   int w[4][4];
 #pragma unroll
   for (int a = 0; a < 4; ++a)
 #pragma unroll
-    for (int b = 0; b < 4; ++b) w[a][b] = img[min(max(y - 2 + a, 0), rows - 1) * cols + min(max(x - 2 + b, 0), cols - 1)];
-  const float nd = L.nextDepth[l][k];
+    for (int b = 0; b < 4; ++b) w[a][b] = img.at(min(max(x - 2 + b, 0), cols - 1), min(max(y - 2 + a, 0), rows - 1));
   float v[3][3];
 #pragma unroll
   for (int dj = 0; dj < 3; ++dj)
@@ -411,7 +435,7 @@
 #pragma unroll
     for (int b = 0; b < 4; ++b) {
       const int u = y - 2 + a, vv = x - 2 + b;
-      if (u >= 0 && u < rows && vv >= 0 && vv < cols) ok = ok && (w[a][b] > 0);
+      ok = ok & (!((u >= 0) & (u < rows) & (vv >= 0) & (vv < cols)) | (w[a][b] > 0));
     }
   if (ok) {
     const int valx = sx, valy = sy;
@@ -421,13 +445,99 @@
   L.mask[l][k] = ok ? 1 : 0;
   L.corres[l][k] = 0u;
 }
+__device__ __forceinline__ void sobel_mask_px(const SobelLevels& L, int l, int x, int y) {
+  const int cols = L.cols[l], rows = L.rows[l];
+  if (x >= cols || y >= rows) return;
+  sobel_mask_at(ImageInMemory<uint8_t>{L.src[l], cols}, L.nextDepth[l][y * cols + x], L, l, x, y);
+}
 __global__ void k_sobel_levels(const SobelLevels L) {
   sobel_mask_px(L, blockIdx.z, blockIdx.x * blockDim.x + threadIdx.x, blockIdx.y * blockDim.y + threadIdx.y);
 }
-__global__ void k_vn_sobel_levels(const VNLevels V, const SobelLevels S) {
-  const int z = blockIdx.z, x = blockIdx.x * blockDim.x + threadIdx.x, y = blockIdx.y * blockDim.y + threadIdx.y;
-  if (z < NUM_PYRS) vmap_nmap_px(V, z, x, y);
-  else sobel_mask_px(S, z - NUM_PYRS, x, y);
+struct PyrStageA {
+  int maps_gx, n_maps, n_sobel;
+  int pyr_gx, n_pyr;
+};
+__global__ void __launch_bounds__(TILE_X * TILE_Y) k_pyr_stage_a(const VNLevels V, const SobelLevels S, const PyrJobs J, const PyrStageA G) {
+  int b = blockIdx.x;
+  if (b < G.n_maps + G.n_sobel) {
+    const bool sobel = b >= G.n_maps;
+    if (sobel) b -= G.n_maps;
+    const int x = (b % G.maps_gx) * TILE_X + threadIdx.x, y = (b / G.maps_gx) * TILE_Y + threadIdx.y;
+    if (sobel) sobel_mask_px(S, 0, x, y);
+    else vmap_nmap_px(V, 0, x, y);
+    return;
+  }
+  b -= G.n_maps + G.n_sobel;
+  const int j = b / G.n_pyr;
+  b -= j * G.n_pyr;
+  pyr_job_px(J, j, (b % G.pyr_gx) * TILE_X + threadIdx.x, (b / G.pyr_gx) * TILE_Y + threadIdx.y);
+}
+constexpr int L2_TW = 16, L2_TH = 4;
+constexpr int L2_PX = L2_TW * L2_TH, L2_LAST_WAVE = TILE_X * TILE_Y - 64;
+static_assert(L2_PX == 64 && (L2_TW + 3) * (L2_TH + 3) <= L2_LAST_WAVE, "one value per thread: the halo'd tile on the first three wavefronts, the plain one on the fourth");
+struct PyrStageB {
+  int tiles_x, n_tiles;
+  int l1_gx, n_maps, n_sobel;
+  int with_sobel;
+  const uint16_t* depth1; uint16_t* depth2;
+  const float* lastDepth1; float* lastDepth2;
+  const uint8_t* lastImage1; uint8_t* lastImage2;
+  const uint8_t* nextImage1; uint8_t* nextImage2;
+};
+__global__ void __launch_bounds__(TILE_X * TILE_Y) k_pyr_stage_b(const VNLevels V, const SobelLevels S, const PyrStageB G) {
+  __shared__ uint16_t depth_s[(L2_TW + 1) * (L2_TH + 1)];
+  __shared__ uint8_t image_s[(L2_TW + 3) * (L2_TH + 3)];
+  __shared__ float last_depth_s[L2_PX];
+  int b = blockIdx.x;
+  if (b >= 2 * G.n_tiles) {
+    b -= 2 * G.n_tiles;
+    const bool sobel = b >= G.n_maps;
+    if (sobel) b -= G.n_maps;
+    const int x = (b % G.l1_gx) * TILE_X + threadIdx.x, y = (b / G.l1_gx) * TILE_Y + threadIdx.y;
+    if (sobel) sobel_mask_px(S, 1, x, y);
+    else vmap_nmap_px(V, 1, x, y);
+    return;
+  }
+  const bool image_kind = b >= G.n_tiles;
+  if (image_kind) b -= G.n_tiles;
+  const int t = threadIdx.y * TILE_X + threadIdx.x;
+  const int x0 = (b % G.tiles_x) * L2_TW, y0 = (b / G.tiles_x) * L2_TH;
+  const int cols = V.cols[2], rows = V.rows[2], scols = V.cols[1], srows = V.rows[1];
+  const int p = t & 63, x = x0 + p % L2_TW, y = y0 + p / L2_TW;
+  const bool inside = x < cols && y < rows;
+  if (!image_kind) {
+    constexpr int RW = L2_TW + 1, RH = L2_TH + 1;
+    if (t < RW * RH) {
+      const int ly = t / RW, lx = t - ly * RW, X = x0 + lx, Y = y0 + ly;
+      if (X < cols && Y < rows) {
+        const uint16_t d = pyr_down_u16_val(G.depth1, scols, srows, X, Y);
+        depth_s[t] = d;
+        if (lx < L2_TW && ly < L2_TH) G.depth2[Y * cols + X] = d;
+      }
+    } else if (t >= L2_LAST_WAVE && inside) {
+      pyr_down_uchar_gauss_px(G.lastImage1, scols, srows, G.lastImage2, x, y);
+    }
+    __syncthreads();
+    if (t < L2_PX) vmap_nmap_at(ImageTile<uint16_t>{depth_s, RW, x0, y0}, V, 2, x, y);
+    return;
+  }
+  constexpr int RW = L2_TW + 3, RH = L2_TH + 3;
+  if (t < RW * RH) {
+    const int ly = t / RW, lx = t - ly * RW, X = x0 - 2 + lx, Y = y0 - 2 + ly;
+    const bool own = lx >= 2 && lx < 2 + L2_TW && ly >= 2 && ly < 2 + L2_TH;
+    if (X >= 0 && Y >= 0 && X < cols && Y < rows && (own || G.with_sobel)) {
+      const uint8_t v = pyr_down_uchar_gauss_val(G.nextImage1, scols, srows, X, Y);
+      image_s[t] = v;
+      if (own) G.nextImage2[Y * cols + X] = v;
+    }
+  } else if (t >= L2_LAST_WAVE && inside) {
+    const float nd = pyr_down_gauss_f_val(G.lastDepth1, scols, srows, x, y);
+    last_depth_s[p] = nd;
+    G.lastDepth2[y * cols + x] = nd;
+  }
+  if (!G.with_sobel) return;
+  __syncthreads();
+  if (t < L2_PX && inside) sobel_mask_at(ImageTile<uint8_t>{image_s, RW, x0 - 2, y0 - 2}, last_depth_s[p], S, 2, x, y);
 }
 
 __device__ __forceinline__ f3 project_point(int x, int y, float z, float invFx, float invFy, float cx, float cy) {
diff --git a/include/ef_hip.h b/include/ef_hip.h
--- a/include/ef_hip.h
+++ b/include/ef_hip.h
@@ -497,6 +497,9 @@
 int ef_op_model_maps(const ef_model_maps_op* args, unsigned* dense_count_left, void* stream);
 int ef_op_sobel_mask(const uint8_t* const* next_image3, const float* const* next_depth3, int cols, int rows, int16_t* const* dIdx3,
                      int16_t* const* dIdy3, uint8_t* const* mask3, uint32_t* const* corres3, void* stream);
+int ef_op_build_pyramids(uint16_t* const* depth3, float* const* last_depth3, uint8_t* const* last_image3, uint8_t* const* next_image3, int cols,
+                         int rows, const ef_intr* intr_level0, float depth_cutoff, int with_sobel, float* const* vmap3, float* const* nmap3,
+                         int16_t* const* dIdx3, int16_t* const* dIdy3, uint8_t* const* mask3, uint32_t* const* corres3, void* stream);
 
 enum ef_linalg_op {
   EF_LINALG_LDLT6 = 0,
```
